# a16z/Lasso

Measured on AMD Instinct MI355X. Metric: prover lookups/sec for SparsePolynomialEvaluationProof, 2^24 AND lookups, higher is better.
Workload: dtype u256 (Montgomery Fr / ed25519 Fq integers)

## Files before the change

### lasso_amd/csrc/lasso_hip.hip

```cpp
#include <hip/hip_runtime.h>
#if defined(__SSE2__)
#include <emmintrin.h>
#endif
#include <mutex>
#include <string>
#include <unordered_map>
#include <vector>
#include <cstring>
#include <cstdio>
#include <cstdlib>
#include <ctime>
#include "../../include/lasso_hip.h"
#include "poly_kernels.cuh"
#include "msm_kernels.cuh"
#include "densify_kernels.cuh"

__global__ void __launch_bounds__(256) k_inner_lr(const fr_t* __restrict__ a, const fr_t* __restrict__ b, size_t half, fr_t* __restrict__ partials) {
  __shared__ RedScratch S;
  fr29 acc[3] = {fr29_zero(), fr29_zero(), fr29_zero()}; uint32_t cnt = 0;
  for (size_t i = blockIdx.x * (size_t)blockDim.x + threadIdx.x; i < half; i += (size_t)gridDim.x * blockDim.x) {
    acc[0] = fr29_weak(fr29_add(acc[0], fr29_mul(fr29_unpack_u(a[i]), fr29_unpack_s(b[half + i]))));
    acc[1] = fr29_weak(fr29_add(acc[1], fr29_mul(fr29_unpack_u(a[half + i]), fr29_unpack_s(b[i]))));
    if ((++cnt & 127u) == 0) { acc[0] = fr29_mul(acc[0], fr29_one_s()); acc[1] = fr29_mul(acc[1], fr29_one_s()); }
  }
  store_block_partials<3>(acc, 2, partials + 2 * (size_t)blockIdx.x, 0, S);
}

static_assert(sizeof(lasso_fr) == 32 && sizeof(fr_t) == 32, "Fr layout");
static_assert(sizeof(lasso_affine) == 64 && sizeof(lasso_point) == 128 && sizeof(ed_point) == 128 && sizeof(niels29) == (MSM_NIELS_ALIGN > 16 ? 128 : 112) && sizeof(pt29) == 144, "curve layouts");

struct EventPair { hipEvent_t a, b; int kid; double bytes, units, units2; bool large; bool counted; };
#define LASSO_PROF_COUNT_SLOTS 4096
struct lasso_ctx {
  int device = 0;
  hipStream_t stream = nullptr;
  std::string err;
  void* d_scratch = nullptr; size_t scratch_cap = 0;
  void* d_pip = nullptr; size_t pip_cap = 0;
  fr_t* d_small = nullptr;
  fr_t* h_small = nullptr;
  size_t small_cap = 0;
  uint32_t* h_flag = nullptr; uint32_t* d_flag = nullptr;
  uint32_t* h_tag = nullptr; uint32_t* d_tag = nullptr;
  bool tagged = true, pending_tagged = false;
  uint32_t pending_groups = 1, pending_K = 0;
  std::vector<lasso_fr> group_tmp;
  uint32_t* mail_h = nullptr; uint32_t* mail_d = nullptr;
  uint32_t seq = 0;
  uint64_t stat_waits = 0; double stat_wait_us = 0;
  fr_t* d_big = nullptr; fr_t* h_big = nullptr; size_t big_cap = 0;
  uint32_t* d_flags = nullptr;
  uint32_t* d_counters = nullptr;
  bool pending = false, defer_next = false; uint32_t pending_seq = 0; size_t pending_count = 0;
  bool ahead_active = false; uint32_t ahead_seq = 0; uint32_t* d_gmail = nullptr;
  bool tail_active = false; uint32_t tail_seq0 = 0, tail_turn = 0, tail_turns = 0; size_t tail_count = 0, tail_final = 0;
  bool tail_unstarted = false;
  uint32_t handover_next = 0;
  size_t ahead_count = 0; bool ahead_tagged = false; uint32_t ahead_groups = 1, ahead_K = 0; bool ahead_bullet = false;
  uint32_t* pmail_h = nullptr; uint32_t* pmail_d = nullptr; uint32_t* d_gpoint = nullptr;
  uint32_t gate_sent = 0;
  bool lay_active = false, lay_tail = false, lay_tagged = false, no_grow = false; uint32_t lay_seq = 0, lay_ell = 0, lay_groups = 1, lay_K = 0, lay_turns = 0; size_t lay_count = 0, lay_final = 0;
  uint32_t prof_mask = 0;
  std::vector<EventPair> events; size_t events_used = 0;
  uint64_t prof_launches[LASSO_K_COUNT] = {0}; double prof_ms[LASSO_K_COUNT] = {0}; double prof_bytes[LASSO_K_COUNT] = {0};
  uint64_t big_launches[LASSO_K_COUNT] = {0}; double big_ms[LASSO_K_COUNT] = {0}; double big_bytes[LASSO_K_COUNT] = {0};
  double prof_units[LASSO_K_COUNT] = {0}; double big_units[LASSO_K_COUNT] = {0};
  double prof_units2[LASSO_K_COUNT] = {0}; double big_units2[LASSO_K_COUNT] = {0};
  double prof_units3[LASSO_K_COUNT] = {0}; double big_units3[LASSO_K_COUNT] = {0};
  uint32_t* d_prof_counts = nullptr;
  void* rccl_comm = nullptr; int rccl_world = 0; int rccl_rank = -1;
  std::unordered_map<void*, size_t> mem_sizes; uint64_t mem_live = 0, mem_peak = 0; std::mutex mem_mu;
};
struct lasso_bases {
  size_t n = 0; niels29* d_table = nullptr;
  lasso_ctx* owner = nullptr;
  niels29* d_mult = nullptr;
  niels29* d_mult8 = nullptr;
  niels29* d_tab8[2] = {nullptr, nullptr};
  bool tab8_failed = false;
  std::mutex tab8_mu;
};

static thread_local std::string g_create_err;
static std::mutex g_ctx_mu; static std::vector<lasso_ctx*> g_ctx_live;
static lasso_ctx* live_or_null(lasso_ctx* c) { std::lock_guard<std::mutex> g(g_ctx_mu); for (lasso_ctx* x : g_ctx_live) if (x == c) return c; return nullptr; }

static int32_t fail(lasso_ctx* c, int32_t code, const std::string& msg) { if (c) c->err = msg; else g_create_err = msg; return code; }
#define HIPCHK(c, call) do { hipError_t e_ = (call); if (e_ != hipSuccess) return fail((c), e_ == hipErrorOutOfMemory ? LASSO_ERR_OOM : LASSO_ERR_HIP, std::string(#call) + ": " + hipGetErrorString(e_)); } while (0)
static inline bool bind_device(lasso_ctx* c) { if (!c) return true; int d = -1; if (hipGetDevice(&d) == hipSuccess && d == c->device) return true; return hipSetDevice(c->device) == hipSuccess; }
#define REQUIRE(c, cond) do { if (!bind_device(c)) return fail((c), LASSO_ERR_HIP, "hipSetDevice failed for the context's device"); \
                              if (!(cond)) return fail((c), LASSO_ERR_INVALID, std::string("invalid argument: ") + #cond); } while (0)

static hipError_t dmalloc(lasso_ctx* c, void** p, size_t bytes) {
  hipError_t e = hipMalloc(p, bytes);
  if (e == hipSuccess && c) { std::lock_guard<std::mutex> g(c->mem_mu); c->mem_sizes[*p] = bytes; c->mem_live += bytes; if (c->mem_live > c->mem_peak) c->mem_peak = c->mem_live; }
  return e;
}
static hipError_t dfree(lasso_ctx* c, void* p) {
  if (c && p) { std::lock_guard<std::mutex> g(c->mem_mu); auto it = c->mem_sizes.find(p); if (it != c->mem_sizes.end()) { c->mem_live -= it->second; c->mem_sizes.erase(it); } }
  return hipFree(p);
}

static int32_t ensure_scratch(lasso_ctx* c, size_t bytes) {
  if (bytes <= c->scratch_cap) return 0;
  if (c->no_grow) return LASSO_ERR_UNSUPPORTED;
  if (c->ahead_active || c->lay_active) return fail(c, LASSO_ERR_INVALID, "a launch is waiting on the device for its challenge: only lasso_result_wait and the post of that challenge are legal until then");
  if (c->d_scratch) { HIPCHK(c, hipStreamSynchronize(c->stream)); HIPCHK(c, dfree(c, c->d_scratch)); c->d_scratch = nullptr; c->scratch_cap = 0; }
  size_t cap = bytes < ((size_t)1 << 22) ? ((size_t)1 << 22) : bytes;
  HIPCHK(c, dmalloc(c, &c->d_scratch, cap)); c->scratch_cap = cap; return 0;
}
static int32_t ensure_pip(lasso_ctx* c, size_t bytes) {
  if (bytes <= c->pip_cap) return 0;
  if (c->no_grow || c->ahead_active || c->lay_active) return LASSO_ERR_UNSUPPORTED;
  if (c->d_pip) { HIPCHK(c, hipStreamSynchronize(c->stream)); HIPCHK(c, dfree(c, c->d_pip)); c->d_pip = nullptr; c->pip_cap = 0; }
  if (dmalloc(c, &c->d_pip, bytes) != hipSuccess) { (void)hipGetLastError(); c->d_pip = nullptr; return LASSO_ERR_UNSUPPORTED; }
  c->pip_cap = bytes; return 0;
}
static int32_t ensure_small(lasso_ctx* c, size_t count) {
  if (count <= c->small_cap) return 0;
  if (c->no_grow) return LASSO_ERR_UNSUPPORTED;
  if (c->ahead_active || c->lay_active) return fail(c, LASSO_ERR_INVALID, "a launch is waiting on the device for its challenge: only lasso_result_wait and the post of that challenge are legal until then");
  HIPCHK(c, hipStreamSynchronize(c->stream));
  if (c->h_small) (void)hipHostFree(c->h_small);
  c->h_small = nullptr; c->d_small = nullptr; c->small_cap = 0;
  size_t cap = count < 4096 ? 4096 : count;
  HIPCHK(c, hipHostMalloc((void**)&c->h_small, cap * sizeof(fr_t), hipHostMallocMapped | hipHostMallocCoherent));
  HIPCHK(c, hipHostGetDevicePointer((void**)&c->d_small, c->h_small, 0));
  if (c->h_tag) (void)hipHostFree(c->h_tag);
  c->h_tag = nullptr; c->d_tag = nullptr;
  HIPCHK(c, hipHostMalloc((void**)&c->h_tag, cap * 48, hipHostMallocMapped | hipHostMallocCoherent));
  memset(c->h_tag, 0, cap * 48);
  HIPCHK(c, hipHostGetDevicePointer((void**)&c->d_tag, c->h_tag, 0));
  c->small_cap = cap; return 0;
}
static int32_t ensure_big(lasso_ctx* c, size_t count) {
  if (count <= c->big_cap) return 0;
  if (c->no_grow) return LASSO_ERR_UNSUPPORTED;
  if (c->ahead_active || c->lay_active) return fail(c, LASSO_ERR_INVALID, "a launch is waiting on the device for its challenge: only lasso_result_wait and the post of that challenge are legal until then");
  HIPCHK(c, hipStreamSynchronize(c->stream));
  if (c->d_big) (void)dfree(c, c->d_big);
  if (c->h_big) (void)hipHostFree(c->h_big);
  c->d_big = nullptr; c->h_big = nullptr; c->big_cap = 0;
  size_t cap = count < 8192 ? 8192 : count;
  HIPCHK(c, dmalloc(c, (void**)&c->d_big, cap * sizeof(fr_t)));
// ... 224 lines not shown
  ncclResult_t r = a->AllGather(d_send, d_recv, bytes, ncclUint8, (ncclComm_t)c->rccl_comm, c->stream);
  if (r != ncclSuccess) return fail(c, LASSO_ERR_HIP, std::string("ncclAllGather: ") + a->GetErrorString(r));
  return 0;
}
int32_t lasso_points_reduce_compress(lasso_ctx* c, const void* d_parts, uint32_t groups, size_t rows, uint8_t* out32) {
  REQUIRE(c, d_parts && out32 && groups >= 1 && rows >= 1);
  int32_t rc = ensure_scratch(c, rows * 32 + 256); if (rc) return rc;
  {
    ProfScope ps(c, LASSO_K_MSM, (double)groups * rows * sizeof(pt29), (double)(groups - 1) * rows);
    hipLaunchKernelGGL(k_points_reduce_compress, dim3(grid_for(rows)), dim3(256), 0, c->stream, (const pt29*)d_parts, groups, rows, (uint32_t*)c->d_scratch);
  }
  HIPCHK(c, hipGetLastError());
  HIPCHK(c, hipMemcpyAsync(out32, c->d_scratch, rows * 32, hipMemcpyDeviceToHost, c->stream));
  HIPCHK(c, hipStreamSynchronize(c->stream));
  return 0;
}

static inline void mail_chunks(uint32_t* mail, uint32_t tag, const uint32_t w[8]) {
  const uint32_t chk = (w[0] ^ w[1] ^ w[2] ^ w[3] ^ w[4] ^ w[5] ^ w[6] ^ w[7]) + tag * 0x9E3779B9u;
#if defined(__SSE2__)
  _mm_store_si128((__m128i*)(mail + 0), _mm_set_epi32((int)w[2], (int)w[1], (int)w[0], (int)tag));
  _mm_store_si128((__m128i*)(mail + 4), _mm_set_epi32((int)w[5], (int)w[4], (int)w[3], (int)tag));
  _mm_store_si128((__m128i*)(mail + 8), _mm_set_epi32((int)chk, (int)w[7], (int)w[6], (int)tag));
#else
  const uint32_t m[12] = {tag, w[0], w[1], w[2], tag, w[3], w[4], w[5], tag, w[6], w[7], chk};
  for (int k : {1, 2, 3, 5, 6, 7, 9, 10, 11}) __atomic_store_n(mail + k, m[k], __ATOMIC_RELAXED);
  for (int k : {0, 4, 8}) __atomic_store_n(mail + k, m[k], __ATOMIC_RELEASE);
#endif
}
static inline void post_mail(lasso_ctx* c, uint32_t tag, const uint32_t w[8]) {
  mail_chunks(c->mail_h, tag, w);
#if defined(__SSE2__)
  _mm_sfence();
#else
  __atomic_thread_fence(__ATOMIC_SEQ_CST);
#endif
}
int32_t lasso_ctx_create(int32_t device, lasso_ctx** out) { return lasso_ctx_create_background(device, 0, out); }
int32_t lasso_ctx_device_uuid(lasso_ctx* c, uint8_t out[16]) {
  REQUIRE(c, c && out);
  hipUUID u; memset(&u, 0, sizeof(u));
  HIPCHK(c, hipDeviceGetUuid(&u, c->device));
  static_assert(sizeof(u.bytes) == 16, "hipUUID");
  memcpy(out, u.bytes, 16); return 0;
}
int32_t lasso_ctx_create_background(int32_t device, int32_t background, lasso_ctx** out) {
  if (!out) return fail(nullptr, LASSO_ERR_INVALID, "out is NULL");
  int n = 0;
  hipError_t e = hipGetDeviceCount(&n);
  if (e != hipSuccess || n == 0) return fail(nullptr, LASSO_ERR_HIP, std::string("no HIP device: ") + hipGetErrorString(e));
  if (device < 0 || device >= n) return fail(nullptr, LASSO_ERR_INVALID, "device index out of range");
  lasso_ctx* c = new lasso_ctx(); c->device = device;
  int prio_lo = 0, prio_hi = 0;
  if ((e = hipSetDevice(device)) == hipSuccess) (void)hipDeviceGetStreamPriorityRange(&prio_lo, &prio_hi);
  if (e != hipSuccess || (e = hipStreamCreateWithPriority(&c->stream, hipStreamNonBlocking, background ? prio_lo : prio_hi)) != hipSuccess) {
    std::string m = hipGetErrorString(e); delete c; return fail(nullptr, LASSO_ERR_HIP, m);
  }
  if (hipMalloc((void**)&c->d_flags, 64) != hipSuccess) { delete c; return fail(nullptr, LASSO_ERR_OOM, "flags alloc"); }
  if (hipMalloc((void**)&c->d_counters, (LASSO_MAX_PTRS + 40) * 4) != hipSuccess || hipMemset(c->d_counters, 0, (LASSO_MAX_PTRS + 40) * 4) != hipSuccess) { delete c; return fail(nullptr, LASSO_ERR_OOM, "counters alloc"); }
  if (hipHostMalloc((void**)&c->h_flag, 256, hipHostMallocMapped | hipHostMallocCoherent) != hipSuccess || hipHostGetDevicePointer((void**)&c->d_flag, c->h_flag, 0) != hipSuccess) { delete c; return fail(nullptr, LASSO_ERR_OOM, "mapped flag alloc"); }
  *c->h_flag = 0;
  { const char* v = getenv("LASSO_TAGGED_RESULTS"); c->tagged = !(v && v[0] == '0'); }
  { const char* v = getenv("LASSO_SEQ_START"); if (v) c->seq = (uint32_t)strtoul(v, nullptr, 0); }
  c->mail_h = c->h_flag + 32; c->mail_d = c->d_flag + 32;
  memset(c->h_flag, 0, 256);
  int32_t rc = ensure_small(c, (size_t)1 << 16); if (rc) { g_create_err = c->err; delete c; return rc; }
  rc = ensure_scratch(c, (size_t)1 << 22); if (rc) { g_create_err = c->err; delete c; return rc; }
  if (dmalloc(c, (void**)&c->d_gmail, 128) != hipSuccess || hipMemset(c->d_gmail, 0, 128) != hipSuccess) { g_create_err = "gmail alloc"; delete c; return LASSO_ERR_OOM; }
  if (hipHostMalloc((void**)&c->pmail_h, LASSO_PMAIL_BYTES, hipHostMallocMapped | hipHostMallocCoherent) != hipSuccess || hipHostGetDevicePointer((void**)&c->pmail_d, c->pmail_h, 0) != hipSuccess) { g_create_err = "point mailbox alloc"; delete c; return LASSO_ERR_OOM; }
  memset(c->pmail_h, 0, LASSO_PMAIL_BYTES);
  if (dmalloc(c, (void**)&c->d_gpoint, LASSO_GPOINT_BYTES) != hipSuccess || hipMemset(c->d_gpoint, 0, LASSO_GPOINT_BYTES) != hipSuccess) { g_create_err = "gpoint alloc"; delete c; return LASSO_ERR_OOM; }
  { std::lock_guard<std::mutex> g(g_ctx_mu); g_ctx_live.push_back(c); }
  *out = c; return 0;
}
int32_t lasso_abort(lasso_ctx* c) {
  REQUIRE(c, c);
  const uint32_t zero8[8] = {0, 0, 0, 0, 0, 0, 0, 0};
  if (c->lay_active && c->pmail_h) for (uint32_t j = 0; j < LASSO_POINT_MAX + 2; j++) mail_chunks(c->pmail_h + 12 * j, LASSO_MAIL_POISON, zero8);
  if (c->tail_active || c->ahead_active || c->lay_active) { mail_chunks(c->mail_h + 12, LASSO_MAIL_POISON, zero8); post_mail(c, LASSO_MAIL_POISON, zero8); }
  (void)hipStreamSynchronize(c->stream);
  (void)hipGetLastError();
  if (c->pmail_h) { memset(c->pmail_h, 0, LASSO_PMAIL_BYTES); c->gate_sent = 0; }
  mail_chunks(c->mail_h + 12, 0, zero8); post_mail(c, 0, zero8);
  c->lay_active = false; c->lay_tail = false; c->no_grow = false;
  c->ahead_active = false; c->ahead_bullet = false; c->tail_unstarted = false; c->handover_next = 0;
  c->tail_active = false; c->pending = false; c->defer_next = false; c->events_used = 0; c->pending_groups = 1; c->pending_K = 0;
  HIPCHK(c, hipMemsetAsync(c->d_counters, 0, (LASSO_MAX_PTRS + 40) * 4, c->stream));
  HIPCHK(c, hipStreamSynchronize(c->stream));
  return 0;
}
void lasso_ctx_destroy(lasso_ctx* c) {
  if (!c) return;
  { std::lock_guard<std::mutex> g(g_ctx_mu); for (size_t i = 0; i < g_ctx_live.size(); i++) if (g_ctx_live[i] == c) { g_ctx_live.erase(g_ctx_live.begin() + i); break; } }
  (void)hipSetDevice(c->device);
  if (c->tail_active || c->pending || c->ahead_active || c->lay_active) (void)lasso_abort(c);
  (void)hipStreamSynchronize(c->stream);
  rccl_release(c);
  for (auto& p : c->events) { (void)hipEventDestroy(p.a); (void)hipEventDestroy(p.b); }
  if (c->d_scratch) (void)hipFree(c->d_scratch);
  if (c->d_pip) (void)hipFree(c->d_pip);
  if (c->d_gmail) (void)hipFree(c->d_gmail);
  if (c->d_gpoint) (void)hipFree(c->d_gpoint);
  if (c->pmail_h) (void)hipHostFree(c->pmail_h);
  if (c->h_small) (void)hipHostFree(c->h_small);
  if (c->h_tag) (void)hipHostFree(c->h_tag);
  if (c->h_flag) (void)hipHostFree(c->h_flag);
  if (c->d_big) (void)hipFree(c->d_big);
  if (c->h_big) (void)hipHostFree(c->h_big);
  if (c->d_flags) (void)hipFree(c->d_flags);
  if (c->d_counters) (void)hipFree(c->d_counters);
  if (c->d_prof_counts) (void)hipFree(c->d_prof_counts);
  (void)hipStreamDestroy(c->stream);
  delete c;
}
const char* lasso_last_error(lasso_ctx* c) { return c ? c->err.c_str() : g_create_err.c_str(); }
void* lasso_stream(lasso_ctx* c) { return c ? (void*)c->stream : nullptr; }
int32_t lasso_alloc(lasso_ctx* c, size_t bytes, void** d_out) { REQUIRE(c, d_out); HIPCHK(c, dmalloc(c, d_out, bytes ? bytes : 1)); return 0; }
int32_t lasso_free(lasso_ctx* c, void* p) { if (!p) return 0; REQUIRE(c, c && !c->ahead_active && !c->lay_active); HIPCHK(c, hipStreamSynchronize(c->stream)); HIPCHK(c, dfree(c, p)); return 0; }
int32_t lasso_mem_stats(lasso_ctx* c, uint64_t* live_bytes, uint64_t* peak_bytes, int32_t reset_peak) {
  REQUIRE(c, c); std::lock_guard<std::mutex> g(c->mem_mu);
  if (live_bytes) *live_bytes = c->mem_live; if (peak_bytes) *peak_bytes = c->mem_peak; if (reset_peak) c->mem_peak = c->mem_live; return 0;
}
int32_t lasso_trim(lasso_ctx* c) {
  REQUIRE(c, c && !c->pending && !c->tail_active && !c->ahead_active && !c->lay_active);
  HIPCHK(c, hipStreamSynchronize(c->stream));
  if (c->d_pip) { HIPCHK(c, dfree(c, c->d_pip)); c->d_pip = nullptr; c->pip_cap = 0; }
  if (c->scratch_cap <= ((size_t)1 << 22)) return 0;
  HIPCHK(c, dfree(c, c->d_scratch)); c->d_scratch = nullptr; c->scratch_cap = 0;
  return ensure_scratch(c, (size_t)1 << 22);
}
int32_t lasso_upload(lasso_ctx* c, void* d, const void* s, size_t n) { REQUIRE(c, d && s && !c->ahead_active && !c->lay_active); HIPCHK(c, hipMemcpyAsync(d, s, n, hipMemcpyHostToDevice, c->stream)); HIPCHK(c, hipStreamSynchronize(c->stream)); return 0; }
int32_t lasso_download(lasso_ctx* c, void* d, const void* s, size_t n) { REQUIRE(c, d && s && !c->ahead_active && !c->lay_active); HIPCHK(c, hipMemcpyAsync(d, s, n, hipMemcpyDeviceToHost, c->stream)); HIPCHK(c, hipStreamSynchronize(c->stream)); return 0; }
int32_t lasso_copy(lasso_ctx* c, void* d, const void* s, size_t n) { REQUIRE(c, d && s); ProfScope ps(c, LASSO_K_MISC, 2.0 * n); HIPCHK(c, hipMemcpyAsync(d, s, n, hipMemcpyDeviceToDevice, c->stream)); return 0; }
int32_t lasso_zero(lasso_ctx* c, void* d, size_t n) { REQUIRE(c, d); HIPCHK(c, hipMemsetAsync(d, 0, n, c->stream)); return 0; }
int32_t lasso_sync(lasso_ctx* c) { REQUIRE(c, c && !c->ahead_active && !c->lay_active); HIPCHK(c, hipStreamSynchronize(c->stream)); return 0; }

int32_t lasso_prof_get_large(lasso_ctx* c, int32_t k, uint64_t* launches, double* ms, double* bytes) {
  REQUIRE(c, k >= 0 && k < LASSO_K_COUNT); prof_flush(c);
  if (launches) *launches = c->big_launches[k]; if (ms) *ms = c->big_ms[k]; if (bytes) *bytes = c->big_bytes[k]; return 0;
}
int32_t lasso_wait_stats(lasso_ctx* c, uint64_t* waits, double* wait_us, int32_t reset) { REQUIRE(c, waits && wait_us); *waits = c->stat_waits; *wait_us = c->stat_wait_us; if (reset) { c->stat_waits = 0; c->stat_wait_us = 0; } return 0; }
int32_t lasso_prof_enable(lasso_ctx* c, int32_t mask) { prof_flush(c); c->prof_mask = (uint32_t)mask; return 0; }
int32_t lasso_prof_reset(lasso_ctx* c) { prof_flush(c); for (int i = 0; i < LASSO_K_COUNT; i++) { c->prof_launches[i] = 0; c->prof_ms[i] = 0; c->prof_bytes[i] = 0; c->big_launches[i] = 0; c->big_ms[i] = 0; c->big_bytes[i] = 0; c->prof_units[i] = 0; c->big_units[i] = 0; c->prof_units2[i] = 0; c->big_units2[i] = 0; c->prof_units3[i] = 0; c->big_units3[i] = 0; } return 0; }
int32_t lasso_prof_get_units(lasso_ctx* c, int32_t k, int32_t large_only, double* units) {
  REQUIRE(c, k >= 0 && k < LASSO_K_COUNT && units); prof_flush(c);
  const bool large = large_only & 1, second = large_only & 2, third = large_only & 4;
  *units = third ? (large ? c->big_units3[k] : c->prof_units3[k]) : second ? (large ? c->big_units2[k] : c->prof_units2[k]) : (large ? c->big_units[k] : c->prof_units[k]); return 0;
}
int32_t lasso_prof_get(lasso_ctx* c, int32_t k, uint64_t* launches, double* ms, double* bytes) {
  REQUIRE(c, k >= 0 && k < LASSO_K_COUNT); prof_flush(c);
  if (launches) *launches = c->prof_launches[k]; if (ms) *ms = c->prof_ms[k]; if (bytes) *bytes = c->prof_bytes[k]; return 0;
}

int32_t lasso_fr_from_u32(lasso_ctx* c, const uint32_t* d_src, size_t n, lasso_fr* d_dst) {
  REQUIRE(c, d_src && d_dst); if (!n) return 0;
  ProfScope ps(c, LASSO_K_MISC, 36.0 * n);
  hipLaunchKernelGGL(k_from_u32, dim3(grid_for(n)), dim3(LASSO_BLOCK), 0, c->stream, d_src, n, (fr_t*)d_dst);
  HIPCHK(c, hipGetLastError()); return 0;
}
__global__ void __launch_bounds__(256) k_subtable_u32(int32_t kind, uint32_t sub, uint32_t log_m, uint32_t log_r, uint32_t* __restrict__ out) {
  const size_t m = (size_t)1 << log_m; const uint32_t bits = log_m / 2, mask = (1u << bits) - 1u;
  for (size_t i = blockIdx.x * (size_t)blockDim.x + threadIdx.x; i < m; i += (size_t)gridDim.x * blockDim.x) {
    const uint32_t r = (uint32_t)i & mask, l = (uint32_t)(i >> bits) & mask;
    uint32_t v;
    if (kind == LASSO_AND) v = l & r;
    else if (kind == LASSO_OR) v = l | r;
    else if (kind == LASSO_XOR) v = l ^ r;
// ... 215 lines not shown
static bool make_eq_inline(const lasso_fr* point, uint32_t ell, const lasso_fr* scale, EqInline& Q) {
  if (ell > 14 || (ell && !point)) return false;
  for (uint32_t j = 0; j < 14; j++) Q.r[j] = j < ell ? to_fr(point + j) : fr_zero();
  Q.scale = scale ? to_fr(scale) : fr_one(); Q.ell = ell; return true;
}
int32_t lasso_sumcheck_cubic_eqw2_begin_eq(lasso_ctx* c, lasso_fr* const* d_A, lasso_fr* const* d_B, uint32_t ncirc, lasso_fr* d_E_out, size_t n, const lasso_fr* point, uint32_t ell, const lasso_fr* scale) {
  REQUIRE(c, d_A && d_B && d_E_out && ncirc >= 1 && ncirc <= LASSO_MAX_PTRS && n >= 2 && (n & (n - 1)) == 0 && !c->pending && ((size_t)1 << ell) == n / 2);
  EqInline Q;
  if (n / 2 <= CUBIC_SMALL_Q || (ell && !point) || ell > 32) return fail(c, LASSO_ERR_UNSUPPORTED, "lasso_sumcheck_cubic_eqw2_begin_eq: tables of 2^7 .. 2^32 entries only");
  uint32_t seq, groups; int32_t rc;
  if (make_eq_inline(point, ell, scale, Q)) rc = cubic_eqw_launch(c, d_A, d_B, ncirc, d_E_out, n, nullptr, 2, &seq, &Q, &groups);
  else { EqPointArg G; G.point = point; G.ell = ell; G.scale = scale ? to_fr(scale) : fr_one(); rc = cubic_eqw_launch(c, d_A, d_B, ncirc, d_E_out, n, nullptr, 2, &seq, nullptr, &groups, false, &G); }
  if (rc) return rc;
  c->pending = true; c->pending_seq = seq; c->pending_count = (size_t)ncirc * 2; c->pending_tagged = c->tagged; c->pending_groups = groups; c->pending_K = 2;
  return 0;
}
int32_t lasso_sumcheck_cubic_tail_begin_eq(lasso_ctx* c, lasso_fr* const* d_A, lasso_fr* const* d_B, uint32_t ncirc, size_t n, const lasso_fr* point, uint32_t ell, const lasso_fr* scale) {
  const uint32_t ho = take_handover(c);
  REQUIRE(c, n >= 2 && ((size_t)1 << ell) == n / 2 && ell <= 9);
  EqInline Q; if (!make_eq_inline(point, ell, scale, Q)) return fail(c, LASSO_ERR_INVALID, "lasso_sumcheck_cubic_tail_begin_eq: bad point");
  return cubic_tail_begin_impl(c, ho, d_A, d_B, ncirc, nullptr, n, nullptr, &Q, false);
}
extern "C++" {
template <class TM>
static int32_t cubic_tail_begin_t(lasso_ctx* c, uint32_t m_stop_arg, lasso_fr* const* d_A, lasso_fr* const* d_B, uint32_t ncirc, const lasso_fr* d_E, size_t n, const lasso_fr* r, const EqInline* eqi, bool ahead, int gate_ell) {
  const uint32_t m_stop = m_stop_arg ? m_stop_arg : 1u;
  const bool gated = gate_ell >= 0;
  REQUIRE(c, d_A && d_B && (d_E || eqi || gated) && ncirc >= 1 && ncirc <= LASSO_MAX_PTRS && n >= ((r || ahead) ? 4u : 2u) && (n & (n - 1)) == 0 && (ahead || gated || !c->pending) && (gated || !c->tail_active) && !c->defer_next && !c->ahead_active && !c->lay_active);
  const size_t q = (r || ahead) ? n / 4 : n / 2;
  REQUIRE(c, q >= 1 && q <= CUBIC_TAIL_Q && (m_stop & (m_stop - 1)) == 0 && m_stop <= 128 && 2 * q > m_stop);
  TM A, B; for (uint32_t i = 0; i < ncirc; i++) { REQUIRE(c, d_A[i] && d_B[i]); A.p[i] = (fr_t*)d_A[i]; B.p[i] = (fr_t*)d_B[i]; }
  int32_t rc = ensure_small(c, (size_t)ncirc * 2 * (m_stop > 2 ? m_stop : 2)); if (rc) return rc;
  uint32_t turns = 0; while (((size_t)m_stop << turns) < 2 * q) turns++;
  const uint32_t seq0 = next_seq(c, turns + 1);
#define LAUNCH_CTAIL(B_, Q_, I_, TE_, R_, EQ_) hipLaunchKernelGGL((k_cubic_tail<B_, Q_, I_, TM, TE_>), dim3(ncirc), dim3(Q_), 0, c->stream, A, B, (const fr_t*)d_E, (uint32_t)q, R_, (const uint32_t*)c->mail_d, c->d_counters, RES(c), seq0, EQ_, m_stop, ahead ? 1u : 0u)
  if (gated) {
    hipLaunchKernelGGL(k_gate_point, dim3(1), dim3(64), 0, c->stream, (const uint32_t*)c->pmail_d, c->d_gpoint, seq0, (uint32_t)gate_ell + 2u, c->pmail_d + LASSO_PMAIL_ACK_WORD); c->gate_sent = seq0;
    EqInlineMem M; M.gp = c->d_gpoint; M.seq = seq0; M.ell = (uint32_t)gate_ell;
    if (q <= 256) LAUNCH_CTAIL(false, 256, true, EqInlineMem, fr_zero(), M); else LAUNCH_CTAIL(false, 512, true, EqInlineMem, fr_zero(), M);
    HIPCHK(c, hipGetLastError());
    c->lay_active = true; c->lay_tail = true; c->lay_seq = seq0; c->lay_ell = (uint32_t)gate_ell; c->lay_turns = turns; c->lay_count = (size_t)ncirc * 2; c->lay_final = (size_t)ncirc * 2 * m_stop; c->lay_tagged = c->tagged;
    return 0;
  }
  if (eqi) { if (q <= 256) LAUNCH_CTAIL(false, 256, true, EqInline, fr_zero(), *eqi); else LAUNCH_CTAIL(false, 512, true, EqInline, fr_zero(), *eqi); }
  else if (q <= 256) { if (r || ahead) LAUNCH_CTAIL(true, 256, false, EqNone, r ? to_fr(r) : fr_zero(), EqNone()); else LAUNCH_CTAIL(false, 256, false, EqNone, fr_zero(), EqNone()); }
  else { if (r || ahead) LAUNCH_CTAIL(true, 512, false, EqNone, r ? to_fr(r) : fr_zero(), EqNone()); else LAUNCH_CTAIL(false, 512, false, EqNone, fr_zero(), EqNone()); }
  HIPCHK(c, hipGetLastError());
  c->tail_active = true; c->tail_seq0 = seq0; c->tail_turn = 0; c->tail_turns = turns; c->tail_count = (size_t)ncirc * 2; c->tail_final = (size_t)ncirc * 2 * m_stop;
  if (ahead) { c->tail_unstarted = true; return 0; }
  c->pending = true; c->pending_seq = seq0; c->pending_count = c->tail_count; c->pending_tagged = c->tagged;
  return 0;
}
}
static int32_t cubic_tail_begin_impl(lasso_ctx* c, uint32_t m_stop, lasso_fr* const* d_A, lasso_fr* const* d_B, uint32_t ncirc, const lasso_fr* d_E, size_t n, const lasso_fr* r, const EqInline* eqi, bool ahead, int gate_ell) {
  return ncirc <= 8 ? cubic_tail_begin_t<MutPtrTable8>(c, m_stop, d_A, d_B, ncirc, d_E, n, r, eqi, ahead, gate_ell) : cubic_tail_begin_t<MutPtrTable>(c, m_stop, d_A, d_B, ncirc, d_E, n, r, eqi, ahead, gate_ell);
}
static bool gate_free(lasso_ctx* c) { return !c->gate_sent || __atomic_load_n(c->pmail_h + LASSO_PMAIL_ACK_WORD, __ATOMIC_ACQUIRE) == c->gate_sent; }
int32_t lasso_layer_ahead_ok(lasso_ctx* c) { static const bool off = [] { const char* v = getenv("LASSO_LAYER_AHEAD"); return v && v[0] == '0'; }(); return c && !off && c->pmail_d && c->d_gpoint ? 1 : 0; }
int32_t lasso_sumcheck_cubic_eqw2_begin_eq_ahead(lasso_ctx* c, lasso_fr* const* d_A, lasso_fr* const* d_B, uint32_t ncirc, lasso_fr* d_E_out, size_t n, uint32_t ell) {
  REQUIRE(c, d_A && d_B && d_E_out && ncirc >= 1 && ncirc <= LASSO_MAX_PTRS && n >= 2 && (n & (n - 1)) == 0 && ell < 48 && ((size_t)1 << ell) == n / 2 && !c->lay_active && !c->ahead_active && !c->defer_next);
  if (!lasso_layer_ahead_ok(c) || n / 2 <= CUBIC_SMALL_Q || ell > 32 || ell > LASSO_POINT_MAX) return fail(c, LASSO_ERR_UNSUPPORTED, "lasso_sumcheck_cubic_eqw2_begin_eq_ahead: tables of 2^7 .. 2^32 entries only");
  if (!gate_free(c)) return fail(c, LASSO_ERR_UNSUPPORTED, "lasso_sumcheck_cubic_eqw2_begin_eq_ahead: the previous point gate has not consumed its message yet");
  uint32_t seq, groups;
  c->no_grow = true;
  const int32_t rc = cubic_eqw_launch(c, d_A, d_B, ncirc, d_E_out, n, nullptr, 2, &seq, nullptr, &groups, false, nullptr, (int)ell);
  c->no_grow = false;
  if (rc == LASSO_ERR_UNSUPPORTED) return fail(c, rc, "lasso_sumcheck_cubic_eqw2_begin_eq_ahead: a buffer would have to grow while kernels are in flight");
  if (rc) return rc;
  HIPCHK(c, hipGetLastError());
  c->lay_active = true; c->lay_tail = false; c->lay_seq = seq; c->lay_ell = ell; c->lay_count = (size_t)ncirc * 2; c->lay_tagged = c->tagged; c->lay_groups = groups; c->lay_K = 2;
  return 0;
}
int32_t lasso_sumcheck_cubic_tail_begin_eq_ahead(lasso_ctx* c, lasso_fr* const* d_A, lasso_fr* const* d_B, uint32_t ncirc, size_t n, uint32_t ell) {
  const uint32_t ho = take_handover(c);
  REQUIRE(c, n >= 2 && ell <= 9 && ((size_t)1 << ell) == n / 2);
  if (!lasso_layer_ahead_ok(c)) return fail(c, LASSO_ERR_UNSUPPORTED, "lasso_sumcheck_cubic_tail_begin_eq_ahead: switched off");
  if (!gate_free(c)) return fail(c, LASSO_ERR_UNSUPPORTED, "lasso_sumcheck_cubic_tail_begin_eq_ahead: the previous point gate has not consumed its message yet");
  c->no_grow = true;
  const int32_t rc = cubic_tail_begin_impl(c, ho, d_A, d_B, ncirc, nullptr, n, nullptr, nullptr, false, (int)ell);
  c->no_grow = false;
  if (rc == LASSO_ERR_UNSUPPORTED) return fail(c, rc, "lasso_sumcheck_cubic_tail_begin_eq_ahead: a buffer would have to grow while kernels are in flight");
  return rc;
}
static void point_mail(lasso_ctx* c, uint32_t ell, const lasso_fr* point, const lasso_fr* scale, uint32_t ctrl) {
  const uint32_t zero8[8] = {0, 0, 0, 0, 0, 0, 0, 0}; const fr_t one = fr_one();
  for (uint32_t j = 0; j < ell; j++) mail_chunks(c->pmail_h + 12 * j, c->lay_seq, point ? (const uint32_t*)(point + j) : zero8);
  mail_chunks(c->pmail_h + 12 * ell, c->lay_seq, scale ? (const uint32_t*)scale : one.v);
  const uint32_t ctl[8] = {ctrl, 0, 0, 0, 0, 0, 0, 0};
  mail_chunks(c->pmail_h + 12 * (ell + 1), c->lay_seq, ctl);
#if defined(__SSE2__)
  _mm_sfence();
#else
  __atomic_thread_fence(__ATOMIC_SEQ_CST);
#endif
}
int32_t lasso_point_post(lasso_ctx* c, const lasso_fr* point, uint32_t ell, const lasso_fr* scale) {
  REQUIRE(c, c && c->lay_active && ell == c->lay_ell && (point || !ell) && !c->pending && !c->tail_active && !c->ahead_active);
  point_mail(c, ell, point, scale, 0u);
  c->lay_active = false;
  if (c->lay_tail) {
    c->tail_active = true; c->tail_seq0 = c->lay_seq; c->tail_turn = 0; c->tail_turns = c->lay_turns; c->tail_count = c->lay_count; c->tail_final = c->lay_final; c->tail_unstarted = false;
    c->pending = true; c->pending_seq = c->lay_seq; c->pending_count = c->lay_count; c->pending_tagged = c->lay_tagged; c->pending_groups = 1; c->pending_K = 0;
  } else {
    c->pending = true; c->pending_seq = c->lay_seq; c->pending_count = c->lay_count; c->pending_tagged = c->lay_tagged; c->pending_groups = c->lay_groups; c->pending_K = c->lay_K;
  }
  c->lay_tail = false;
  return 0;
}
int32_t lasso_point_cancel(lasso_ctx* c) {
  REQUIRE(c, c && c->lay_active);
  point_mail(c, c->lay_ell, nullptr, nullptr, 1u);
  c->lay_active = false; c->lay_tail = false;
  return 0;
}
int32_t lasso_sumcheck_cubic_tail_begin_ahead(lasso_ctx* c, lasso_fr* const* d_A, lasso_fr* const* d_B, uint32_t ncirc, const lasso_fr* d_E, size_t n) {
  const uint32_t ho = take_handover(c);
  REQUIRE(c, d_E);
  return cubic_tail_begin_impl(c, ho, d_A, d_B, ncirc, d_E, n, nullptr, nullptr, true);
}
int32_t lasso_tail_handover_next(lasso_ctx* c, uint32_t m_stop) {
  REQUIRE(c, c && (m_stop & (m_stop - 1)) == 0 && m_stop <= 128);
  c->handover_next = m_stop <= 1 ? 0 : m_stop; return 0;
}
int32_t lasso_sumcheck_linear_tail_begin(lasso_ctx* c, const lasso_fr* const* d_src, uint32_t alpha, const lasso_fr* d_E, size_t n, const lasso_fr* r) {
  const uint32_t ho = take_handover(c);
  REQUIRE(c, d_src && d_E && alpha >= 1 && alpha <= LASSO_MAX_PTRS && n >= (r ? 4u : 2u) && (n & (n - 1)) == 0 && !c->pending && !c->tail_active && !c->defer_next && !ho && !c->ahead_active);
  const size_t q = r ? n / 4 : n / 2;
  REQUIRE(c, q >= 1 && q <= CUBIC_TAIL_Q);
  PtrTable Src; for (uint32_t i = 0; i < alpha; i++) { REQUIRE(c, d_src[i]); Src.p[i] = (const fr_t*)d_src[i]; }
  int32_t rc = ensure_small(c, (size_t)alpha * 3); if (rc) return rc;
  uint32_t turns = 0; while (((size_t)1 << turns) < 2 * q) turns++;
  const uint32_t seq0 = next_seq(c, turns + 1);
#define LAUNCH_LTAIL(B_, Q_, R_) hipLaunchKernelGGL((k_linear_tail<B_, Q_>), dim3(alpha), dim3(Q_), 0, c->stream, Src, (const fr_t*)d_E, (uint32_t)q, R_, (const uint32_t*)c->mail_d, c->d_counters, RES(c), seq0)
  if (q <= 256) { if (r) LAUNCH_LTAIL(true, 256, to_fr(r)); else LAUNCH_LTAIL(false, 256, fr_zero()); }
  else { if (r) LAUNCH_LTAIL(true, 512, to_fr(r)); else LAUNCH_LTAIL(false, 512, fr_zero()); }
  HIPCHK(c, hipGetLastError());
  c->tail_active = true; c->tail_seq0 = seq0; c->tail_turn = 0; c->tail_turns = turns; c->tail_count = (size_t)alpha * 2; c->tail_final = alpha;
  c->pending = true; c->pending_seq = seq0; c->pending_count = c->tail_count; c->pending_tagged = c->tagged;
  return 0;
}
int32_t lasso_sumcheck_cubic_tail_next(lasso_ctx* c, const lasso_fr* r) {
  REQUIRE(c, r && c->tail_active && !c->pending);
  const fr_t rr = to_fr(r);
  if (c->tail_unstarted) {
    c->tail_unstarted = false;
    post_mail(c, c->tail_seq0, rr.v);
    c->pending = true; c->pending_seq = c->tail_seq0; c->pending_count = c->tail_count; c->pending_tagged = c->tagged;
    return 0;
  }
  c->tail_turn++;
  const uint32_t tn = c->tail_seq0 + c->tail_turn;
  post_mail(c, tn, rr.v);
  const size_t cnt = c->tail_turn == c->tail_turns ? c->tail_final : c->tail_count;
  if (cnt) { c->pending = true; c->pending_seq = c->tail_seq0 + c->tail_turn; c->pending_count = cnt; c->pending_tagged = c->tagged; }
  if (c->tail_turn == c->tail_turns) c->tail_active = false;
  return 0;
}
uint32_t lasso_sumcheck_tail_capacity(void) { static const uint32_t q = [] { const char* v = getenv("LASSO_TAIL_Q"); const long x = v ? atol(v) : 0; return (uint32_t)(x == 256 ? 256 : CUBIC_TAIL_Q); }(); return q; }
int32_t lasso_defer_next(lasso_ctx* c) { REQUIRE(c, !c->pending && !c->defer_next); c->defer_next = true; return 0; }
int32_t lasso_result_wait(lasso_ctx* c, lasso_fr* out, size_t count) {
  REQUIRE(c, out && c->pending && count == c->pending_count);
  c->pending = false;
  { const uint32_t g = c->pending_groups, K = c->pending_K; c->pending_groups = 1; c->pending_K = 0; return wait_flag(c, c->pending_seq, count, out, c->pending_tagged, g, K); }
}
int32_t lasso_sumcheck_linear_eqw_round(lasso_ctx* c, const lasso_fr* const* d_polys, uint32_t alpha, const lasso_fr* d_E, size_t n, lasso_fr* out) {
  REQUIRE(c, d_polys && d_E && out && alpha >= 1 && alpha <= LASSO_MAX_PTRS && n >= 2 && (n & (n - 1)) == 0);
  PtrTable P; for (uint32_t i = 0; i < alpha; i++) { REQUIRE(c, d_polys[i]); P.p[i] = (const fr_t*)d_polys[i]; }
  const size_t half = n / 2; const unsigned ny = alpha, nx = grid_for(half, cubic_nx_cap(ny));
  int32_t rc = ensure_small(c, (size_t)alpha * 3); if (rc) return rc;
  rc = ensure_scratch(c, (size_t)nx * ny * 3 * sizeof(fr_t)); if (rc) return rc;
  const uint32_t seq = next_seq(c);
  {
    ProfScope ps(c, LASSO_K_COMBINE, 32.0 * n * (alpha + 1.0));
    hipLaunchKernelGGL(k_dot_eqw_lb, dim3(nx * ny), dim3(LASSO_BLOCK), 0, c->stream, P, nx, ny, (const fr_t*)d_E, half, (fr_t*)c->d_scratch, c->d_counters, RES(c), seq);
  }
  HIPCHK(c, hipGetLastError());
  return wait_flag(c, seq, (size_t)alpha * 3, out, c->tagged);
}
int32_t lasso_sumcheck_linear_eqw_round_fused(lasso_ctx* c, lasso_fr* const* d_polys, uint32_t alpha, const lasso_fr* d_E, size_t n, const lasso_fr* r, lasso_fr* out) {
  return lasso_sumcheck_linear_eqw_round_fused_from(c, (const lasso_fr* const*)d_polys, d_polys, alpha, d_E, n, r, out);
}
int32_t lasso_sumcheck_linear_eqw_round_fused_from(lasso_ctx* c, const lasso_fr* const* d_src, lasso_fr* const* d_polys, uint32_t alpha, const lasso_fr* d_E, size_t n, const lasso_fr* r, lasso_fr* out) {
  REQUIRE(c, d_src && d_polys && d_E && r && out && alpha >= 1 && alpha <= LASSO_MAX_PTRS && n >= 4 && (n & (n - 1)) == 0);
  MutPtrTable P; PtrTable Src; for (uint32_t i = 0; i < alpha; i++) { REQUIRE(c, d_polys[i] && d_src[i]); P.p[i] = (fr_t*)d_polys[i]; Src.p[i] = (const fr_t*)d_src[i]; }
  const size_t q = n / 4; const unsigned ny = alpha, nx = grid_for(q, cubic_nx_cap(ny));
  int32_t rc = ensure_small(c, (size_t)alpha * 3); if (rc) return rc;
  rc = ensure_scratch(c, (size_t)nx * ny * 3 * sizeof(fr_t)); if (rc) return rc;
  const uint32_t seq = next_seq(c);
  {
    ProfScope ps(c, LASSO_K_BIND, 48.0 * n * (alpha + 1.0));
    hipLaunchKernelGGL(k_dot_eqw_fused<false>, dim3(nx * ny), dim3(LASSO_BLOCK), 0, c->stream, Src, P, nx, ny, (const fr_t*)d_E, q, to_fr(r), (fr_t*)c->d_scratch, c->d_counters, RES(c), seq);
  }
  HIPCHK(c, hipGetLastError());
  return wait_flag(c, seq, (size_t)alpha * 3, out, c->tagged);
}
// ... 787 lines not shown
```

### lasso_amd/csrc/poly_kernels.cuh

```cuda
#pragma once
#define LASSO_MAIL_POISON 0xFFFFFFFFu
#include <hip/hip_runtime.h>
#include "fr.cuh"
#include "fr29.cuh"

#ifndef LASSO_MAX_PTRS
#define LASSO_MAX_PTRS 136
#endif
#define LASSO_BLOCK 256
#define LASSO_MAX_ALPHA 32

struct PtrTable { const fr_t* p[LASSO_MAX_PTRS]; };
struct MutPtrTable { fr_t* p[LASSO_MAX_PTRS]; };
struct PtrTable8 { const fr_t* p[8]; };
struct MutPtrTable8 { fr_t* p[8]; };
struct StrategyDev { int kind; uint32_t c, log_m, log_r, alpha; };
struct WeightTable { fr_t w[LASSO_MAX_ALPHA]; };

struct RedScratch { int32_t rows[LASSO_BLOCK * 27]; int64_t strips[8 * 27]; int64_t cols[27]; };
template <int NV>
__device__ __forceinline__ void block_columns(const fr29* vals, RedScratch& S) {
  const uint32_t t = threadIdx.x;
  __syncthreads();
#pragma unroll
// ... 45 lines not shown
#pragma unroll
      for (int k = 0; k < 4; k++) __hip_atomic_store(o + k, (uint64_t)v.v[2 * k] | ((uint64_t)v.v[2 * k + 1] << 32), __ATOMIC_RELAXED, __HIP_MEMORY_SCOPE_AGENT);
      return;
    }
#endif
    out[slot] = v;
  }
}
__device__ __forceinline__ bool mail_valid(const lasso_u32x4& c0, const lasso_u32x4& c1, const lasso_u32x4& c2, uint32_t tag) {
  return c0.x == tag && c1.x == tag && c2.x == tag && c2.w == (c0.y ^ c0.z ^ c0.w ^ c1.y ^ c1.z ^ c1.w ^ c2.y ^ c2.z) + tag * 0x9E3779B9u;
}
__device__ __forceinline__ bool mail_wait(const uint32_t* mailbox, uint32_t tag, uint64_t t_end, fr_t& chal) {
  const lasso_u32x4* m4 = reinterpret_cast<const lasso_u32x4*>(mailbox);
  lasso_u32x4 c0, c1, c2; uint32_t spins = 0;
  for (;;) {
#ifndef LASSO_NO_POLL_FENCE
    __builtin_amdgcn_fence(__ATOMIC_ACQUIRE, "");
#else
    asm volatile("" ::: "memory");
#endif
    c0 = __builtin_nontemporal_load(m4); c1 = __builtin_nontemporal_load(m4 + 1); c2 = __builtin_nontemporal_load(m4 + 2);
    if (mail_valid(c0, c1, c2, tag)) break;
    if (c0.x == LASSO_MAIL_POISON || ((++spins & 63u) == 0 && wall_clock64() > t_end)) return false;
  }
  chal.v[0] = c0.y; chal.v[1] = c0.z; chal.v[2] = c0.w; chal.v[3] = c1.y; chal.v[4] = c1.z; chal.v[5] = c1.w; chal.v[6] = c2.y; chal.v[7] = c2.z;
  return true;
}
__global__ void __launch_bounds__(64) k_gate(const uint32_t* mail, uint32_t* gmail, uint32_t seq, uint32_t pair) {
  if (threadIdx.x != 0) return;
  const uint64_t t_end = wall_clock64() + 500000000ull;
  fr_t c0, c1;
  bool ok = mail_wait(mail, seq, t_end, c0);
  if (ok && pair) ok = mail_wait(mail + 12, seq, t_end, c1);
  if (ok) {
#pragma unroll
    for (int k = 0; k < 8; k++) { gmail[k] = c0.v[k]; if (pair) gmail[8 + k] = c1.v[k]; }
    gmail[16] = seq;
  } else gmail[17] = seq;
}
__device__ __forceinline__ bool ahead_challenge(const uint32_t* mail, uint32_t* gmail, uint32_t seq, fr_t& r, uint32_t* s_mail) {
  if (threadIdx.x == 0) {
    const uint64_t t_end = wall_clock64() + 500000000ull;
    uint32_t ok = 1, spins = 0;
    if (blockIdx.x == 0) {
      fr_t c;
      if (mail_wait(mail, seq, t_end, c)) {
#pragma unroll
        for (int k = 0; k < 8; k++) gmail[k] = c.v[k];
        __builtin_amdgcn_fence(__ATOMIC_RELEASE, "agent");
        __hip_atomic_store(gmail + 16, seq, __ATOMIC_RELEASE, __HIP_MEMORY_SCOPE_AGENT);
      } else __hip_atomic_store(gmail + 17, seq, __ATOMIC_RELEASE, __HIP_MEMORY_SCOPE_AGENT);
    }
    for (;;) {
      if (__hip_atomic_load(gmail + 16, __ATOMIC_ACQUIRE, __HIP_MEMORY_SCOPE_AGENT) == seq) break;
      if (__hip_atomic_load(gmail + 17, __ATOMIC_ACQUIRE, __HIP_MEMORY_SCOPE_AGENT) == seq || ((++spins & 63u) == 0 && wall_clock64() > t_end + 100000000ull)) { ok = 0; break; }
      __builtin_amdgcn_s_sleep(8);
    }
    if (ok) {
#pragma unroll
      for (int k = 0; k < 8; k++) s_mail[k] = __hip_atomic_load(gmail + k, __ATOMIC_RELAXED, __HIP_MEMORY_SCOPE_AGENT);
    }
    s_mail[8] = ok;
  }
  __syncthreads();
  if (!s_mail[8]) return false;
#pragma unroll
  for (int k = 0; k < 8; k++) r.v[k] = s_mail[k];
  return true;
}
__device__ __forceinline__ bool gated_challenge(const uint32_t* gmail, uint32_t seq, uint32_t words, uint32_t* s_mail) {
  if (threadIdx.x < 17) {
    const uint32_t t = threadIdx.x;
    if (t < words) s_mail[t] = gmail[t];
    if (t == 16) s_mail[16] = (gmail[16] == seq && gmail[17] != seq) ? 1u : 0u;
  }
  __syncthreads();
  return s_mail[16] != 0;
}
#define LASSO_POINT_MAX 40
#define LASSO_GP_TAG (8 * (LASSO_POINT_MAX + 2))
#define LASSO_PMAIL_BYTES 2048
#define LASSO_GPOINT_BYTES 2048
#define LASSO_PMAIL_ACK_WORD 504
__global__ void __launch_bounds__(64) k_gate_point(const uint32_t* pmail, uint32_t* gpoint, uint32_t seq, uint32_t nfr, uint32_t* ack) {
  const uint32_t t = threadIdx.x;
  const uint64_t t_end = wall_clock64() + 500000000ull;
  bool ok = true; fr_t v = fr_zero();
  if (t < nfr) {
    ok = mail_wait(pmail + 12 * t, seq, t_end, v);
    if (ok) {
#pragma unroll
      for (int k = 0; k < 8; k++) gpoint[8 * t + k] = v.v[k];
      if (t == nfr - 1 && v.v[0] != 0) ok = false;
    }
  }
  const bool all_ok = __ballot(!ok) == 0;
  __builtin_amdgcn_fence(__ATOMIC_RELEASE, "agent");
  if (t == 0) { gpoint[LASSO_GP_TAG + (all_ok ? 0 : 1)] = seq; if (ack) __hip_atomic_store(ack, seq, __ATOMIC_RELEASE, __HIP_MEMORY_SCOPE_SYSTEM); }
}
__device__ __forceinline__ bool gate_point_ok(const uint32_t* __restrict__ gp, uint32_t seq) { return gp[LASSO_GP_TAG] == seq && gp[LASSO_GP_TAG + 1] != seq; }
__device__ __forceinline__ fr_t gate_point_fr(const uint32_t* __restrict__ gp, uint32_t j) {
  fr_t r;
#pragma unroll
  for (int k = 0; k < 8; k++) r.v[k] = gp[8 * j + k];
  return r;
}
template <int KMAX>
__device__ __forceinline__ void store_block_partials(const fr29* acc, uint32_t K, fr_t* __restrict__ dst, int shift, RedScratch& S, uint32_t* flag = nullptr, uint32_t seq = 0, size_t slot0 = 0) {
#pragma unroll
  for (int k0 = 0; k0 < KMAX; k0 += 3) if ((uint32_t)k0 < K) {
    fr29 grp[3];
#pragma unroll
    for (int v = 0; v < 3; v++) grp[v] = (k0 + v < KMAX) ? acc[(k0 + v < KMAX) ? k0 + v : 0] : fr29_zero();
    block_columns<3>(grp, S);
    if (threadIdx.x < 3 && k0 + threadIdx.x < K) result_store(dst, slot0 + k0 + threadIdx.x, columns_to_fr(S, threadIdx.x, shift), flag, seq);
  }
}

__device__ __forceinline__ void reduce_partials_row(const fr_t* __restrict__ partials, uint32_t nx, uint32_t K, uint32_t y, fr_t* __restrict__ out, RedScratch& S, uint32_t Kv = 0xffffffffu,
                                                    uint32_t* flag = nullptr, uint32_t seq = 0) {
  if (Kv > K) Kv = K;
  for (uint32_t k0 = 0; k0 < Kv; k0 += 3) {
    fr29 acc[3];
#pragma unroll
    for (int v = 0; v < 3; v++) {
      acc[v] = fr29_zero();
      if (k0 + v < Kv) for (uint32_t x = threadIdx.x; x < nx; x += blockDim.x) acc[v] = fr29_weak(fr29_add(acc[v], fr29_unpack_u(partials[((size_t)y * nx + x) * K + k0 + v])));
    }
    block_columns<3>(acc, S);
    if (threadIdx.x < 3 && k0 + threadIdx.x < Kv) result_store(out, (size_t)y * K + k0 + threadIdx.x, columns_to_fr(S, threadIdx.x, 0), flag, seq);
  }
}
__global__ void __launch_bounds__(LASSO_BLOCK) k_reduce_partials(const fr_t* __restrict__ partials, uint32_t nx, uint32_t K, fr_t* __restrict__ out) {
  __shared__ RedScratch S;
  reduce_partials_row(partials, nx, K, blockIdx.x, out, S);
}

__device__ __forceinline__ void row_done(uint32_t nrows, uint32_t* counters, uint32_t* flag, uint32_t seq);
__device__ __forceinline__ void last_block_reduce(const fr_t* partials, uint32_t nx, uint32_t K, uint32_t y, uint32_t nrows, uint32_t* counters, fr_t* __restrict__ out, RedScratch& S,
                                                  uint32_t* flag, uint32_t seq, uint32_t Kv = 0xffffffffu) {
  __shared__ uint32_t is_last;
  if (threadIdx.x == 0) {
#ifdef LASSO_PLAIN_PARTIALS
    __builtin_amdgcn_fence(__ATOMIC_RELEASE, "agent");
#endif
    asm volatile("s_waitcnt vmcnt(0)" ::: "memory");
    uint32_t ticket = __hip_atomic_fetch_add(&counters[y], 1u, __ATOMIC_RELAXED, __HIP_MEMORY_SCOPE_AGENT);
    uint32_t last = (ticket == nx - 1) ? 1u : 0u;
    if (last) { __builtin_amdgcn_fence(__ATOMIC_ACQUIRE, "agent"); counters[y] = 0; }
    is_last = last;
  }
  __syncthreads();
  if (!is_last) return;
  reduce_partials_row(partials, nx, K, y, out, S, Kv, flag, seq);
  row_done(nrows, counters, flag, seq);
}

__global__ void __launch_bounds__(LASSO_BLOCK) k_bind_top(MutPtrTable polys, size_t half, fr_t r) {
  fr_t* __restrict__ z = polys.p[blockIdx.y];
  const fr29 rs = fr29_unpack_s(r);
  for (size_t i = blockIdx.x * (size_t)blockDim.x + threadIdx.x; i < half; i += (size_t)gridDim.x * blockDim.x) {
    const fr29 lo = fr29_unpack_u(z[i]), hi = fr29_unpack_u(z[i + half]);
    z[i] = fr29_store(fr29_add(lo, fr29_mul(fr29_sub(hi, lo), rs)));
  }
}

__device__ __forceinline__ void cubic_terms(const fr29& a0, const fr29& a1, const fr29& b0, const fr29& b1, const fr29& c0, const fr29& c1, fr29& t0, fr29& t2, fr29& t3) {
  t0 = fr29_mul(c0, fr29_mul(a0, b0));
  const fr29 da = fr29_sub(a1, a0), db = fr29_sub(b1, b0), dc = fr29_sub(c1, c0);
  const fr29 a2 = fr29_weak(fr29_add(a1, da)), b2 = fr29_weak(fr29_add(b1, db)), c2 = fr29_weak(fr29_add(c1, dc));
  t2 = fr29_mul(c2, fr29_mul(a2, b2));
  const fr29 a3 = fr29_add(a2, da), b3 = fr29_weak(fr29_add(b2, db)), c3 = fr29_add(c2, dc);
  t3 = fr29_mul(c3, fr29_mul(a3, b3));
}
struct CubicGrid { uint32_t bx, by, nx, ny; };
__device__ __forceinline__ CubicGrid cubic_grid(uint32_t nx, uint32_t ny) {
  CubicGrid g; g.nx = nx; g.ny = ny;
  const uint32_t b = blockIdx.x;
  if ((nx & 7u) == 0) { const uint32_t grp = b / (8 * ny), r = b - grp * 8 * ny; g.by = r >> 3; g.bx = grp * 8 + (r & 7u); }
  else { g.bx = b % nx; g.by = b / nx; }
  return g;
// ... 96 lines not shown
    fr29 p = one_s;
    for (uint32_t j = 0; j < lb; j++) { const bool bit = (x >> (lb - 1 - j)) & 1u; const fr29 rs = fr29_unpack_s(eq_point_r(Q, hb + j)); p = fr29_mul(bit ? rs : fr29_sub(one_s, rs), p); }
    T.lo_s[x] = p;
    T.lo_u[x] = fr29_mul(p, fr29_unpack_u(fr_one()));
  }
  __syncthreads();
  return true;
}
__device__ __forceinline__ bool eq_inline_build(const EqInline& Q, EqInlineTables& T) { return eq_inline_build_t(Q, T); }
__device__ __forceinline__ bool eq_inline_build(const EqInlineMem& Q, EqInlineTables& T) { return eq_inline_build_t(Q, T); }
__device__ __forceinline__ fr29 eq_inline_s(const EqInlineTables& T, uint32_t lb, size_t x) { return fr29_mul(T.hi_s[x >> lb], T.lo_s[x & ((1u << lb) - 1u)]); }
struct EqGlobal { const fr_t* hi; const fr_t* lo; uint32_t lo_bits; uint32_t ell; const uint32_t* gp; uint32_t seq; };
__device__ __forceinline__ bool eq_inline_build(const EqGlobal& Q, EqInlineTables&) { return Q.gp == nullptr || gate_point_ok(Q.gp, Q.seq); }
__device__ __forceinline__ bool eq_inline_build(const EqNone&, EqInlineTables&) { return true; }
template <class TE> __device__ __forceinline__ bool eq_gate_ok(const TE&) { return true; }
template <> __device__ __forceinline__ bool eq_gate_ok<EqNone>(const EqNone& Q) { return Q.gp == nullptr || gate_point_ok(Q.gp, Q.seq); }
__device__ __forceinline__ fr29 eq_inline_value(const EqInline&, const EqInlineTables& T, uint32_t lb, size_t i, bool write, fr_t* __restrict__ E_out) {
  if (write) E_out[i] = fr29_store(fr29_mul(T.hi_s[i >> lb], T.lo_u[i & ((1u << lb) - 1u)]));
  return eq_inline_s(T, lb, i);
}
__device__ __forceinline__ fr29 eq_inline_value(const EqInlineMem&, const EqInlineTables& T, uint32_t lb, size_t i, bool write, fr_t* __restrict__ E_out) {
  if (write) E_out[i] = fr29_store(fr29_mul(T.hi_s[i >> lb], T.lo_u[i & ((1u << lb) - 1u)]));
  return eq_inline_s(T, lb, i);
}
__device__ __forceinline__ fr29 eq_inline_value(const EqGlobal& Q, const EqInlineTables&, uint32_t, size_t i, bool write, fr_t* __restrict__ E_out) {
  const fr_t mem = fr29_store(fr29_mul(fr29_unpack_u(Q.hi[i >> Q.lo_bits]), fr29_unpack_s(Q.lo[i & (((size_t)1 << Q.lo_bits) - 1)])));
  if (write) E_out[i] = mem;
  return fr29_unpack_s(mem);
}
__device__ __forceinline__ fr29 eq_inline_value(const EqNone&, const EqInlineTables&, uint32_t, size_t, bool, fr_t* __restrict__) { return fr29_zero(); }
__device__ __forceinline__ fr_t fr_load_nt(const fr_t* p) {
  const lasso_u32x4* q = reinterpret_cast<const lasso_u32x4*>(p);
  const lasso_u32x4 x = __builtin_nontemporal_load(q), y = __builtin_nontemporal_load(q + 1);
  fr_t r; r.v[0] = x.x; r.v[1] = x.y; r.v[2] = x.z; r.v[3] = x.w; r.v[4] = y.x; r.v[5] = y.y; r.v[6] = y.z; r.v[7] = y.w; return r;
}
template <int NT, bool EQI = false, class TP = PtrTable, class TE = EqInline, bool NTL = false>
__global__ void __launch_bounds__(LASSO_BLOCK) k_cubic_eqw_lb(TP A, TP B, uint32_t nx, uint32_t ny, const fr_t* __restrict__ E, size_t half, fr_t* __restrict__ partials, uint32_t* counters,
                                                               fr_t* __restrict__ out, uint32_t* flag, uint32_t seq, uint32_t pipeline, TE EQ = TE(), fr_t* __restrict__ E_out = nullptr) {
  __shared__ RedScratch S;
  __shared__ EqInlineTables ET;
  const CubicGrid g = cubic_grid(nx, ny);
  const uint32_t elb = EQ.ell / 2;
  if constexpr (EQI) { if (!eq_inline_build(EQ, ET)) return; } else { if (!eq_gate_ok(EQ)) return; }
  const fr_t* __restrict__ a = A.p[g.by];
  const fr_t* __restrict__ b = B.p[g.by];
  fr29 e[3] = {fr29_zero(), fr29_zero(), fr29_zero()}; uint32_t cnt = 0;
  fr29_acc w0 = fr29_acc_zero(), w1 = fr29_acc_zero();
  const size_t stride = (size_t)nx * blockDim.x;
  size_t i = g.bx * (size_t)blockDim.x + threadIdx.x;
  if (NT == 3) {
    for (; i < half; i += stride) {
      fr29 t0, t2, t3;
      cubic_eqw_terms(fr29_unpack_u(a[i]), fr29_unpack_u(a[i + half]), fr29_unpack_u(b[i]), fr29_unpack_u(b[i + half]), fr29_unpack_s(E[i]), t0, t2, t3); CUBIC_ACCUMULATE(e, t0, t2, t3, cnt);
    }
  } else if (!pipeline) {
    for (; i < half; i += stride) {
      const fr29 es = fr29_unpack_s(E[i]), b0 = fr29_unpack_u(b[i]), b1 = fr29_unpack_u(b[i + half]);
      const fr29 g0 = fr29_mul(fr29_unpack_u(a[i]), es), g1 = fr29_mul(fr29_unpack_u(a[i + half]), es);
      fr29_mul_acc(w0, b0, g0); fr29_mul_acc(w1, fr29_sub(g1, g0), fr29_sub(b1, b0));
      if (++cnt == 3) { fr29_acc_carry(w0); fr29_acc_carry(w1); cnt = 0; }
    }
  } else if (i < half) {
#define LB_LD(ptr) (NTL ? fr_load_nt(ptr) : *(ptr))
    fr_t a0 = LB_LD(a + i), a1 = LB_LD(a + i + half), b0m = LB_LD(b + i), b1m = LB_LD(b + i + half), em = EQI ? fr_zero() : E[i];
    for (;;) {
      const size_t in = i + stride; const bool more = in < half;
      const size_t ip = more ? in : i;
      const fr_t na0 = LB_LD(a + ip), na1 = LB_LD(a + ip + half), nb0 = LB_LD(b + ip), nb1 = LB_LD(b + ip + half), ne = EQI ? fr_zero() : E[ip];
#undef LB_LD
      fr29 es;
      if (EQI) es = eq_inline_value(EQ, ET, elb, i, g.by == 0, E_out);
      else es = fr29_unpack_s(em);
      const fr29 b0 = fr29_unpack_u(b0m), b1 = fr29_unpack_u(b1m);
      const fr29 g0 = fr29_mul(fr29_unpack_u(a0), es), g1 = fr29_mul(fr29_unpack_u(a1), es);
      fr29_mul_acc(w0, b0, g0); fr29_mul_acc(w1, fr29_sub(g1, g0), fr29_sub(b1, b0));
      if (++cnt == 3) { fr29_acc_carry(w0); fr29_acc_carry(w1); cnt = 0; }
      if (!more) break;
      a0 = na0; a1 = na1; b0m = nb0; b1m = nb1; em = ne; i = in;
    }
  }
  if (NT == 2) { fr29_acc_carry(w0); fr29_acc_carry(w1); e[0] = fr29_acc_reduce(w0); e[1] = fr29_acc_reduce(w1); }
  cubic_epilogue(e, g, partials, counters, out, flag, seq, S, 5, NT);
}
template <int NT, bool WIDE = false, class TM = MutPtrTable, bool AHEAD = false>
#ifdef LASSO_FUSED_WAVES
__attribute__((amdgpu_waves_per_eu(LASSO_FUSED_WAVES, LASSO_FUSED_WAVES)))
#endif
__global__ void __launch_bounds__(LASSO_BLOCK) k_cubic_eqw_fused(TM A, TM B, uint32_t nx, uint32_t ny, const fr_t* __restrict__ E, size_t q, fr_t r,
                                                                  fr_t* __restrict__ partials, uint32_t* counters, fr_t* __restrict__ out, uint32_t* flag, uint32_t seq,
                                                                  const uint32_t* gmail = nullptr, const uint32_t* mail = nullptr) {
  __shared__ RedScratch S;
  const CubicGrid g = cubic_grid(nx, ny);
  fr_t* __restrict__ a = A.p[g.by];
  fr_t* __restrict__ b = B.p[g.by];
  if constexpr (AHEAD) {
    __shared__ uint32_t s_mail[17];
    if (mail) {
      if (!ahead_challenge(mail, const_cast<uint32_t*>(gmail), seq, r, s_mail)) return;
    } else {
      if (!gated_challenge(gmail, seq, 8, s_mail)) return;
#pragma unroll
      for (int k = 0; k < 8; k++) r.v[k] = s_mail[k];
    }
  }
  const fr29 rs = fr29_unpack_s(r);
  fr29 e[3] = {fr29_zero(), fr29_zero(), fr29_zero()}; uint32_t cnt = 0;
  fr29_acc w0 = fr29_acc_zero(), w1 = fr29_acc_zero();
  for (size_t i = g.bx * (size_t)blockDim.x + threadIdx.x; i < q; i += (size_t)nx * blockDim.x) {
    const fr29 a0 = NT == 2 ? bind29_semi(a[i], a[i + 2 * q], rs) : bind29(a[i], a[i + 2 * q], rs), a1 = NT == 2 ? bind29_semi(a[i + q], a[i + 3 * q], rs) : bind29(a[i + q], a[i + 3 * q], rs);
    a[i] = fr29_pack(a0); a[i + q] = fr29_pack(a1);
    const fr29 b0 = NT == 2 ? bind29_semi(b[i], b[i + 2 * q], rs) : bind29(b[i], b[i + 2 * q], rs), b1 = NT == 2 ? bind29_semi(b[i + q], b[i + 3 * q], rs) : bind29(b[i + q], b[i + 3 * q], rs);
    b[i] = fr29_pack(b0); b[i + q] = fr29_pack(b1);
    fr29 t0, t2, t3;
    if (NT == 3) { cubic_eqw_terms(a0, a1, b0, b1, fr29_unpack_s(E[i]), t0, t2, t3); CUBIC_ACCUMULATE(e, t0, t2, t3, cnt); }
    else if (!WIDE) { cubic_eqw_terms2(a0, a1, b0, b1, fr29_unpack_s(E[i]), t0, t2); CUBIC_ACCUMULATE2(e, t0, t2, cnt); }
    else {
      const fr29 es = fr29_unpack_s(E[i]);
      const fr29 g0 = fr29_mul(a0, es), g1 = fr29_mul(a1, es);
      fr29_mul_acc(w0, b0, g0); fr29_mul_acc(w1, fr29_sub(g1, g0), fr29_sub(b1, b0));
      if (++cnt == 3) { fr29_acc_carry(w0); fr29_acc_carry(w1); cnt = 0; }
    }
  }
  if (WIDE && NT == 2) { fr29_acc_carry(w0); fr29_acc_carry(w1); e[0] = fr29_acc_reduce(w0); e[1] = fr29_acc_reduce(w1); }
  cubic_epilogue(e, g, partials, counters, out, flag, seq, S, 5, NT);
}
template <bool BIND, int NT, class TM = MutPtrTable>
__global__ void __launch_bounds__(LASSO_BLOCK) k_cubic_eqw_small(TM A, TM B, const fr_t* __restrict__ E, uint32_t q, fr_t r, uint32_t* counters, fr_t* __restrict__ out,
                                                                  uint32_t* flag, uint32_t seq) {
  __shared__ fr29 bound[2][128];
  __shared__ fr29 ge[128];
  __shared__ int32_t rows[192 * 9];
  __shared__ int64_t cols[27];
  const uint32_t t = threadIdx.x, y = blockIdx.x, m = 2 * q;
  const fr29 rs = fr29_unpack_s(r);
  for (uint32_t item = t; item < 2 * m; item += LASSO_BLOCK) {
    const uint32_t p = item / m, i = item - p * m;
    fr_t* dst = p == 0 ? A.p[y] : B.p[y];
    fr29 v;
    if (BIND) { v = bind29(dst[i], dst[i + m], rs); dst[i] = fr29_pack(v); } else v = fr29_unpack_u(dst[i]);
    bound[p][i] = v;
  }
  __syncthreads();
  if (t < m) ge[t] = fr29_mul(bound[0][t], fr29_unpack_s(E[t < q ? t : t - q]));
  __syncthreads();
  const uint32_t x = t >> 6, i = t & 63;
  if (x < NT) {
    fr29 term = fr29_zero();
    if (i < q) {
      const fr29 g0 = ge[i], g1 = ge[i + q], b0 = bound[1][i], b1 = bound[1][i + q];
      if (x == 0) term = fr29_mul(b0, g0);
      else if (NT == 2) term = fr29_mul(fr29_sub(g1, g0), fr29_sub(b1, b0));
      else {
        const fr29 dg = fr29_sub(g1, g0), db = fr29_sub(b1, b0);
        const fr29 g2 = fr29_weak(fr29_add(g1, dg)), b2 = fr29_weak(fr29_add(b1, db));
        term = x == 1 ? fr29_mul(b2, g2) : fr29_mul(fr29_add(b2, db), fr29_weak(fr29_add(g2, dg)));
      }
    }
#pragma unroll
    for (int k = 0; k < 9; k++) rows[t * 9 + k] = term.v[k];
  }
  __syncthreads();
  if (t < 9 * NT) {
    const uint32_t v = t / 9, k = t - v * 9;
    int64_t sum = 0;
    for (uint32_t j = 0; j < 64; j++) sum += rows[(v * 64 + j) * 9 + k];
    cols[t] = sum;
// ... 729 lines not shown
```

### lasso_amd/host/prover.hpp

```cpp
#pragma once
#include <array>
#include <functional>
#include <map>
#include <memory>
#include <string>
#include <vector>
#include "field_host.hpp"
#include "field52.hpp"
#include "hashes.hpp"
#include "../../include/lasso_prover.h"

#include <chrono>
#include <cstdio>
#include <cstdlib>

namespace lasso {

struct Trace {
  static bool on() { static const bool v = [] { const char* e = getenv("LASSO_TRACE"); return e && e[0] == '1'; }(); return v; }
  static bool mem() { static const bool v = [] { const char* e = getenv("LASSO_TRACE"); return e && e[0] == '3'; }(); return v; }
  const char* name; lasso_ctx* ctx; std::chrono::steady_clock::time_point t0; static int& depth() { static thread_local int d = 0; return d; }
  uint64_t w0 = 0; double wus0 = 0; uint64_t live0 = 0;
  Trace(const char* n, lasso_ctx* c) : name(n), ctx(c) {
    if (on()) { t0 = std::chrono::steady_clock::now(); depth()++; if (ctx) lasso_wait_stats(ctx, &w0, &wus0, 0); }
    if (mem() && ctx) { uint64_t pk = 0; lasso_mem_stats(ctx, &live0, &pk, 1); depth()++; }
  }
  ~Trace() {
    if (mem() && ctx) {
      uint64_t live = 0, pk = 0; lasso_mem_stats(ctx, &live, &pk, 1); depth()--;
      fprintf(stderr, "[mem] %*s%s: live at entry %.2f GB, peak inside %.2f GB, live at exit %.2f GB\n", 2 * depth(), "", name, live0 / 1e9, pk / 1e9, live / 1e9);
    }
    if (!on()) return;
    if (ctx) lasso_sync(ctx);
    depth()--;
    double ms = std::chrono::duration<double, std::milli>(std::chrono::steady_clock::now() - t0).count();
    uint64_t w1 = 0; double wus1 = 0; if (ctx) lasso_wait_stats(ctx, &w1, &wus1, 0);
    fprintf(stderr, "[trace] %*s%s: time.busy=%.3fms (device hand-offs %llu, host spinning %.3fms)\n", 2 * depth(), "", name, ms, (unsigned long long)(w1 - w0), (wus1 - wus0) * 1e-3);
  }
};

struct HostClock {
  static bool on() { static const bool v = [] { const char* e = getenv("LASSO_TRACE"); return e && e[0] == '2'; }(); return v; }
  static std::map<std::string, double>& buckets() { static thread_local std::map<std::string, double> b; return b; }
  const char* name; std::chrono::steady_clock::time_point t0;
  explicit HostClock(const char* n) : name(n) { if (on()) t0 = std::chrono::steady_clock::now(); }
  ~HostClock() { if (on()) buckets()[name] += std::chrono::duration<double, std::milli>(std::chrono::steady_clock::now() - t0).count(); }
  static void dump() { if (!on()) return; for (auto& kv : buckets()) fprintf(stderr, "[host] %-28s %.3f ms\n", kv.first.c_str(), kv.second); buckets().clear(); }
};
struct Error : std::runtime_error { using std::runtime_error::runtime_error; };
#define LASSO_REQUIRE(c) do { if (!(c)) throw Error(std::string("lasso prover: requirement failed: ") + #c); } while (0)

#define LASSO_HOST_TOPS_MAX_PTRS 128
inline size_t next_pow2(size_t n) { size_t p = 1; while (p < n) p <<= 1; return p; }
inline bool is_pow2(size_t n) { return n && !(n & (n - 1)); }
inline size_t ceil_log2(size_t n) { size_t k = 0; while (((size_t)1 << k) < n) k++; return k; }

typedef int32_t (*lasso_allgather_fn)(void* user, const void* send, void* recv, size_t bytes);
struct Comm {
  size_t rank = 0, world = 1; lasso_allgather_fn fn = nullptr; void* user = nullptr;
  bool shared_device = false;
  bool sharded() const { return world > 1; }
  size_t log_world() const { size_t k = 0; while (((size_t)1 << k) < world) k++; return k; }
  void allgather(const void* send, void* recv, size_t bytes) const {
    if (world == 1) { memcpy(recv, send, bytes); return; }
    if (!fn || fn(user, send, recv, bytes) != 0) throw std::runtime_error("lasso prover: all-gather failed");
  }
  void sum(std::vector<lasso_fr>& v) const {
    if (world == 1 || v.empty()) return;
    std::vector<lasso_fr> all(v.size() * world);
    allgather(v.data(), all.data(), v.size() * sizeof(lasso_fr));
    for (size_t i = 0; i < v.size(); i++) { Sc acc = Sc::zero(); for (size_t g = 0; g < world; g++) acc += Sc::from_abi(all[g * v.size() + i]); v[i] = acc.abi(); }
  }
  Sc eq_low(const ScVec& point) const {
    const size_t p = log_world(); Sc f = Sc::one();
    for (size_t b = 0; b < p; b++) { const Sc& rv = point[point.size() - 1 - b]; f *= ((rank >> b) & 1) ? rv : (Sc::one() - rv); }
    return f;
  }
};

class Dev {
  mutable std::multimap<size_t, void*> pool_;
  mutable std::map<void*, size_t> live_;
  mutable size_t in_use_ = 0, in_use_peak_ = 0;
  int device_ = 0;
  mutable lasso_ctx* side_ = nullptr;

 public:
  lasso_ctx* ctx = nullptr;
  Comm comm;
  bool capacity = [] { const char* e = getenv("LASSO_CAPACITY"); return e && e[0] == '1'; }();
  bool throughput = false;
  bool no_ahead() const { static const bool keep = [] { const char* e = getenv("LASSO_THROUGHPUT_AHEAD"); return e && e[0] == '1'; }(); return throughput && !keep; }
// ... 453 lines not shown
  size_t s_loc, m_loc;
  std::vector<DBufU32> dim_u32;
  DBuf combined_l_variate_polys, combined_log_m_variate_polys;
  size_t nv_l, nv_m;
  bool compact = false;
  std::vector<DBufU32> read_u32; std::vector<uint32_t> read_max;
  const lasso_fr* dim(size_t i) const { LASSO_REQUIRE(!compact); return combined_l_variate_polys.p + i * s_loc; }
  const lasso_fr* read(size_t i) const { LASSO_REQUIRE(!compact); return combined_l_variate_polys.p + (C + i) * s_loc; }
  const uint32_t* block_u32(size_t b) const { return b < C ? dim_u32[b].p : read_u32[b - C].p; }
  uint32_t block_max(size_t b) const { return b < C ? (uint32_t)(m - 1) : read_max[b - C]; }
  void lift_block(size_t b, lasso_fr* d_tmp) const { dev->chk(lasso_fr_from_u32(dev->ctx, block_u32(b), s_loc, d_tmp), "lasso_fr_from_u32"); }
  const lasso_fr* final_(size_t i) const { return combined_log_m_variate_polys.p + i * m_loc; }

  static std::unique_ptr<DensifiedRepresentation> from_lookup_indices(const Dev& d, const uint64_t* indices, size_t n_lookups, size_t C, size_t log_m) {
    Trace tr_all("DensifiedRepresentation.from_lookup_indices", d.ctx);
    auto D = std::make_unique<DensifiedRepresentation>();
    D->dev = &d; D->C = C; D->s = next_pow2(n_lookups); D->log_m = log_m; D->m = (size_t)1 << log_m;
    const size_t s = D->s, m = D->m, P = d.comm.world;
    if (d.comm.sharded() && (s < 2 * P || m < 2 * P)) throw Error("slab sharding needs at least 2 lookups and 2 table entries per rank");
    D->s_loc = s / P; D->m_loc = m / P;
    size_t n_l = next_pow2(2 * C * s), n_m = next_pow2(C) * m;
    D->nv_l = ceil_log2(n_l); D->nv_m = ceil_log2(n_m);
    if (d.comm.sharded() && (((size_t)1 << (D->nv_m - D->nv_m / 2)) < P || ((size_t)1 << (D->nv_l - D->nv_l / 2)) < P)) throw Error("slab sharding needs every Hyrax matrix to have at least one column per rank");
    D->compact = d.capacity && !capacity_compact_off() && D->s_loc >= capacity_leafless_min() && s >= ((size_t)1 << (D->nv_l - D->nv_l / 2));
    D->combined_log_m_variate_polys = DBuf(d, n_m / P);
    if (!D->compact) D->combined_l_variate_polys = DBuf(d, n_l / P);
    if (!D->compact && n_l > 2 * C * s) d.chk(lasso_zero(d.ctx, D->combined_l_variate_polys.p + 2 * C * D->s_loc, (n_l - 2 * C * s) / P * sizeof(lasso_fr)), "lasso_zero");
    if (n_m > C * m) d.chk(lasso_zero(d.ctx, D->combined_log_m_variate_polys.p + C * D->m_loc, (n_m - C * m) / P * sizeof(lasso_fr)), "lasso_zero");
    DBufU64 d_idx(d, indices, n_lookups * C);
    DBuf tmp_dim, tmp_read; if (D->compact) { tmp_dim = DBuf(d, D->s_loc); tmp_read = DBuf(d, D->s_loc); }
    for (size_t i = 0; i < C; i++) {
      DBufU32 d_access(d, D->s_loc);
      lasso_fr* dim_out = D->compact ? tmp_dim.p : D->combined_l_variate_polys.p + i * D->s_loc;
      lasso_fr* read_out = D->compact ? tmp_read.p : D->combined_l_variate_polys.p + (C + i) * D->s_loc;
      d.chk(lasso_densify_dim_slab(d.ctx, d_idx.p, n_lookups, C, i, s, (uint32_t)log_m, (uint32_t)P, (uint32_t)d.comm.rank, d_access.p, dim_out, read_out, D->combined_log_m_variate_polys.p + i * D->m_loc), "lasso_densify_dim");
      D->dim_u32.push_back(std::move(d_access));
      if (D->compact) {
        DBufU32 r32(d, D->s_loc); uint32_t mx = 0;
        d.chk(lasso_fr_to_u32(d.ctx, tmp_read.p, D->s_loc, r32.p, &mx), "lasso_fr_to_u32");
        D->read_u32.push_back(std::move(r32)); D->read_max.push_back(mx);
      }
    }
    if (D->compact) { tmp_dim.release(); tmp_read.release(); }
    if (d.capacity) (void)lasso_trim(d.ctx);
    return D;
  }
  SparsePolynomialCommitment commit(const SparsePolyCommitmentGens& gens) const {
    Trace tr_all("DensifiedRepresentation.commit", dev->ctx);
    SparsePolynomialCommitment c;
    if (!compact) c.l_variate_polys_commitment = hyrax_commit(*dev, combined_l_variate_polys.p, nv_l, gens.gens_combined_l_variate);
    else {
      const size_t L = (size_t)1 << (nv_l / 2), R = (size_t)1 << (nv_l - nv_l / 2), rows_per = s / R;
      PolyCommitment& pc = c.l_variate_polys_commitment; pc.rows = L; pc.compressed.reserve(32 * L);
      DBuf tmp(*dev, s_loc);
      for (size_t b = 0; b < 2 * C; b++) {
        PolyCommitment part;
        if (!dev->comm.sharded()) part = hyrax_commit_rows(*dev, nullptr, rows_per, R, gens.gens_combined_l_variate, block_u32(b), block_max(b));
        else { lift_block(b, tmp.p); part = hyrax_commit_rows(*dev, tmp.p, rows_per, R, gens.gens_combined_l_variate); }
        pc.compressed.insert(pc.compressed.end(), part.compressed.begin(), part.compressed.end());
      }
      if (2 * C * rows_per < L) {
        dev->chk(lasso_zero(dev->ctx, tmp.p, (R / dev->comm.world) * sizeof(lasso_fr)), "lasso_zero");
        PolyCommitment zero_row = hyrax_commit_rows(*dev, tmp.p, 1, R, gens.gens_combined_l_variate);
        for (size_t r = 2 * C * rows_per; r < L; r++) pc.compressed.insert(pc.compressed.end(), zero_row.compressed.begin(), zero_row.compressed.end());
      }
      tmp.release();
    }
    c.log_m_variate_polys_commitment = hyrax_commit(*dev, combined_log_m_variate_polys.p, nv_m, gens.gens_combined_log_m_variate);
    c.s = s; c.log_m = log_m; c.m = m; return c;
  }
};

class Prover {
  const Dev& d; const Strategy S; DensifiedRepresentation& dense; const SparsePolyCommitmentGens& gens; ProofTranscript& t; RandomTape& tape;
  size_t alpha, s, m, nv_derefs;
  size_t P, lgP, s_loc, m_loc;
  std::vector<DBuf> tables;
  DBuf combined_E;
  const lasso_fr* E(size_t i) const { return combined_E.p + i * s_loc; }
  std::vector<DBuf> tail_bufs;
  std::vector<DBuf> side_keep;
  static size_t tail_q() { static const size_t q = lasso_sumcheck_tail_capacity(); return q; }
  struct LazyEq { bool on = false; std::vector<lasso_fr> rr; lasso_fr scale; lasso_fr* d_table = nullptr; } lazy_eq;
  struct LayerAhead { bool on = false, tail = false; std::vector<lasso_fr*> A, B; lasso_fr* d_table = nullptr; size_t len = 0, m_stop = 1; uint32_t ell = 0; } layer_ahead;
  std::function<void()> next_layer_hook;
  static bool tail_switched_off() { static const bool off = [] { const char* v = getenv("LASSO_CUBIC_TAIL"); return v && v[0] == '0'; }(); return off; }
  bool layer_ahead_ok() { return P == 1 && !d.no_ahead() && !eq_inline_off() && !tail_switched_off() && lasso_layer_ahead_ok(d.ctx) == 1; }
  void enqueue_layer_ahead(const std::vector<lasso_fr*>& A, const std::vector<lasso_fr*>& B, size_t len, lasso_fr* d_table) {
    layer_ahead.on = false;
    if (!layer_ahead_ok() || len < 4) return;
    const size_t k = A.size(); const uint32_t ell = (uint32_t)ceil_log2(len / 2);
    LayerAhead la; la.A = A; la.B = B; la.d_table = d_table; la.len = len; la.ell = ell;
    int32_t rc;
    if (len / 2 <= tail_q()) {
      if (ell > 9) return;
      const size_t m0 = host_m_stop(k); la.m_stop = (m0 >= 2 && m0 < len) ? m0 : 1; la.tail = true;
      if (la.m_stop > 1) d.chk(lasso_tail_handover_next(d.ctx, (uint32_t)la.m_stop), "lasso_tail_handover_next");
      rc = lasso_sumcheck_cubic_tail_begin_eq_ahead(d.ctx, la.A.data(), la.B.data(), (uint32_t)k, len, ell);
    } else {
      if (ell > 32 || len / 2 <= 64) return;
      rc = lasso_sumcheck_cubic_eqw2_begin_eq_ahead(d.ctx, la.A.data(), la.B.data(), (uint32_t)k, d_table, len, ell);
    }
    if (rc == LASSO_ERR_UNSUPPORTED) return;
    d.chk(rc, "lasso_sumcheck_cubic_*_begin_eq_ahead");
    la.on = true; layer_ahead = std::move(la);
  }
  static bool eq_inline_off() { static const bool v = [] { const char* e = getenv("LASSO_EQ_INLINE"); return e && e[0] == '0'; }(); return v; }
  static bool side_off() { static const bool v = [] { const char* e = getenv("LASSO_SIDE_STREAM"); return e && e[0] == '0'; }(); return v; }

 public:
  std::vector<uint8_t> proof_bytes;
  Prover(const Dev& d_, const Strategy& S_, DensifiedRepresentation& dense_, const SparsePolyCommitmentGens& gens_, ProofTranscript& t_, RandomTape& tape_)
      : d(d_), S(S_), dense(dense_), gens(gens_), t(t_), tape(tape_) {
    alpha = S.num_memories(); s = dense.s; m = dense.m; LASSO_REQUIRE(S.C() == dense.C && S.M() == dense.m);
    P = d.comm.world; lgP = d.comm.log_world(); s_loc = dense.s_loc; m_loc = dense.m_loc;
  }

  void eq_evals_local(const ScVec& point, lasso_fr* d_out) {
    LASSO_REQUIRE(point.size() >= lgP);
    std::vector<lasso_fr> rr; for (size_t i = 0; i + lgP < point.size(); i++) rr.push_back(point[i].abi());
    if (P == 1) { d.chk(lasso_eq_evals(d.ctx, rr.data(), (uint32_t)rr.size(), d_out), "lasso_eq_evals"); return; }
    lasso_fr sc = d.comm.eq_low(point).abi();
    d.chk(lasso_eq_evals_scaled(d.ctx, rr.data(), (uint32_t)rr.size(), &sc, d_out), "lasso_eq_evals_scaled");
  }
  void eq_half_local(const ScVec& point, lasso_fr* d_out) {
    LASSO_REQUIRE(point.size() >= lgP);
    if (point.size() == lgP) return;
    std::vector<lasso_fr> rr; for (size_t i = 1; i + lgP < point.size(); i++) rr.push_back(point[i].abi());
    Sc scale = Sc::one() - point[0]; if (P > 1) scale *= d.comm.eq_low(point);
    lasso_fr sc = scale.abi();
    d.chk(lasso_eq_evals_scaled(d.ctx, rr.data(), (uint32_t)rr.size(), &sc, d_out), "lasso_eq_evals_scaled");
  }
  void eq_half_lazy(const ScVec& point, lasso_fr* d_out) {
    LASSO_REQUIRE(point.size() >= lgP);
    lazy_eq.on = false;
    if (point.size() == lgP) return;
    lazy_eq.rr.clear(); for (size_t i = 1; i + lgP < point.size(); i++) lazy_eq.rr.push_back(point[i].abi());
    Sc scale = Sc::one() - point[0]; if (P > 1) scale *= d.comm.eq_low(point);
    lazy_eq.scale = scale.abi(); lazy_eq.d_table = d_out; lazy_eq.on = true;
  }
  std::vector<lasso_fr*> gather_tail(const std::vector<lasso_fr*>& polys) {
    const size_t k = polys.size();
    std::vector<lasso_fr> mine(k), all(k * P), col(P);
    d.chk(lasso_read_heads(d.ctx, (const lasso_fr* const*)polys.data(), (uint32_t)k, mine.data()), "lasso_read_heads");
    d.comm.allgather(mine.data(), all.data(), k * sizeof(lasso_fr));
    std::vector<lasso_fr*> out;
    for (size_t i = 0; i < k; i++) {
      for (size_t g = 0; g < P; g++) col[g] = all[g * k + i];
      tail_bufs.emplace_back(d, P);
      d.chk(lasso_upload(d.ctx, tail_bufs.back().p, col.data(), P * sizeof(lasso_fr)), "lasso_upload");
      out.push_back(tail_bufs.back().p);
    }
    return out;
  }

  void arbitrary_rounds(size_t rounds, size_t len, std::vector<lasso_fr*>& polys, size_t combined_degree, bool reduce, SumcheckProof& proof, ScVec& r_out, const std::vector<const uint32_t*>* first_u32 = nullptr) {
    std::vector<const lasso_fr*> cp(polys.begin(), polys.begin() + alpha);
    for (size_t round = 0; round < rounds; round++) {
      std::vector<lasso_fr> ev(combined_degree + 1);
      if (S.spark()) d.chk(lasso_sumcheck_combine_round(d.ctx, &S.abi, cp.data(), polys[alpha], len, (uint32_t)combined_degree, ev.data()), "lasso_sumcheck_combine_round");
      else if (round == 0 && first_u32) d.chk(lasso_sumcheck_combine_round_lt_u32(d.ctx, &S.abi, first_u32->data(), polys[alpha], len, (uint32_t)combined_degree, ev.data()), "lasso_sumcheck_combine_round_lt_u32");
      else d.chk(lasso_sumcheck_combine_round_lt_scaled(d.ctx, &S.abi, cp.data(), polys[alpha], len, (uint32_t)combined_degree, ev.data()), "lasso_sumcheck_combine_round_lt_scaled");
      if (reduce) d.comm.sum(ev);
      ScVec evals; for (auto& e : ev) evals.push_back(Sc::from_abi(e));
      UniPoly up = UniPoly::from_evals(evals);
      up.append_to_transcript(t, "poly");
      Sc r_j = t.challenge_scalar("challenge_nextround"); r_out.push_back(r_j);
      lasso_fr rj = r_j.abi();
      d.chk(lasso_bind_top(d.ctx, polys.data(), (uint32_t)polys.size(), len, &rj), "lasso_bind_top");
      len /= 2;
      proof.compressed_polys.push_back(up.compress());
    }
  }
  void linear_rounds(size_t rounds, size_t len, std::vector<lasso_fr*>& polys, const lasso_fr* d_E, const ScVec& point, size_t v0, bool reduce, Sc& s_run, SumcheckProof& proof, ScVec& r_out,
                     const std::vector<const lasso_fr*>* src = nullptr, std::vector<lasso_fr>* tail_heads = nullptr, const std::vector<const uint32_t*>* src_u32 = nullptr) {
    if (tail_heads) tail_heads->clear();
    if (!rounds) return;
    if (src && rounds < 2) {
      for (size_t i = 0; i < polys.size(); i++) d.chk(lasso_copy(d.ctx, polys[i], (*src)[i], len * sizeof(lasso_fr)), "lasso_copy");
      src = nullptr;
    }
    const ScVec w = S.weights();
    ScVec inv(rounds); bool degenerate = false;
    {
// ... 202 lines not shown
    std::vector<H4> A, B, Aw;
    if (!vec) {
      A.resize(k * m); B.resize(k * m); Aw.resize(k * m);
      for (size_t c = 0; c < k; c++) { const H4 w = h4_from(coeffs[c].v); for (size_t i = 0; i < m; i++) { A[c * m + i] = h4_from(a[c][i].v); B[c * m + i] = h4_from(b[c][i].v); Aw[c * m + i] = h4_mul(A[c * m + i], w); } }
    }
    size_t stride = m;
    for (size_t j = 0; j < rounds_left; j++) {
      const size_t h = m / 2;
      H4 e0 = h4_zero(), e2 = h4_zero(), e3 = h4_zero();
#ifdef LASSO_HOST_IFMA
      if (vec) v52->sums(h, e0, e2, e3); else
#endif
      for (size_t i = 0; i < h; i++) {
        H4 t0 = h4_zero(), t2 = h4_zero(), t3 = h4_zero();
        for (size_t c = 0; c < k; c++) {
          const H4 *pa = &Aw[c * stride], *pb = &B[c * stride];
          const H4 da = h4_sub(pa[i + h], pa[i]), db = h4_sub(pb[i + h], pb[i]), a2 = h4_add(pa[i + h], da), b2 = h4_add(pb[i + h], db), a3 = h4_add(a2, da), b3 = h4_add(b2, db);
          t0 = h4_add(t0, h4_mul(pa[i], pb[i])); t2 = h4_add(t2, h4_mul(a2, b2)); t3 = h4_add(t3, h4_mul(a3, b3));
        }
        const H4 dc = h4_sub(C[i + h], C[i]), c2 = h4_add(C[i + h], dc), c3 = h4_add(c2, dc);
        e0 = h4_add(e0, h4_mul(t0, C[i])); e2 = h4_add(e2, h4_mul(t2, c2)); e3 = h4_add(e3, h4_mul(t3, c3));
      }
      static const H4 inv2 = h4_from(Sc::from_u64(2).inverse().v), inv6 = h4_from(Sc::from_u64(6).inverse().v);
      const H4 e1 = h4_sub(h4_from(e.v), e0);
      const H4 t32 = h4_sub(e3, h4_add(h4_add(e2, e2), e2)), t11 = h4_add(h4_add(e1, e1), e1);
      const H4 k3 = h4_mul(h4_sub(h4_add(t32, t11), e0), inv6);
      const H4 k2 = h4_sub(h4_mul(h4_add(h4_sub(e2, h4_add(e1, e1)), e0), inv2), h4_add(h4_add(k3, k3), k3));
      const H4 k1 = h4_sub(h4_sub(h4_sub(e1, e0), k2), k3);
      UniPoly poly; poly.coeffs = {to_sc(e0), to_sc(k1), to_sc(k2), to_sc(k3)};
      poly.append_to_transcript(t, "poly");
      const Sc r_j = t.challenge_scalar("challenge_nextround"); r_out.push_back(r_j);
      e = poly.evaluate(r_j);
      proof.compressed_polys.push_back(poly.compress());
      const H4 rj = h4_from(r_j.v);
#ifdef LASSO_HOST_IFMA
      if (vec) v52->bind(h, rj); else
#endif
      {
        for (size_t c = 0; c < k; c++) for (H4* arr : {&A[c * stride], &B[c * stride], &Aw[c * stride]}) for (size_t i = 0; i < h; i++) arr[i] = h4_add(arr[i], h4_mul(rj, h4_sub(arr[i + h], arr[i])));
        for (size_t i = 0; i < h; i++) C[i] = h4_add(C[i], h4_mul(rj, h4_sub(C[i + h], C[i])));
      }
      m = h;
    }
    heads.resize(2 * k);
#ifdef LASSO_HOST_IFMA
    if (vec) { std::vector<H4> hh; v52->heads(hh); for (size_t c = 0; c < 2 * k; c++) heads[c] = to_sc(hh[c]).abi(); return; }
#endif
    for (size_t c = 0; c < k; c++) { heads[c] = to_sc(A[c * stride]).abi(); heads[k + c] = to_sc(B[c * stride]).abi(); }
  }
  void cubic_rounds(size_t rounds, size_t len, std::vector<lasso_fr*>& A, std::vector<lasso_fr*>& B, const lasso_fr* d_E, const ScVec& rand, size_t v0, const ScVec& coeffs, bool reduce, Sc& s_run,
                    Sc& e, SumcheckProof& proof, ScVec& r_out, std::vector<lasso_fr>* heads_out = nullptr, const LeafLayer* leaf = nullptr) {
    const size_t k = leaf ? 2 * leaf->mems.size() : A.size();
    if (heads_out) heads_out->clear();
    std::unique_ptr<HostClock> hpro(new HostClock("layer transition: sumcheck prologue"));
    LayerAhead pre = std::move(layer_ahead); layer_ahead.on = false;
    std::function<void()> hook = std::move(next_layer_hook); next_layer_hook = nullptr;
    if (!rounds) { if (pre.on) d.chk(lasso_point_cancel(d.ctx), "lasso_point_cancel"); return; }
    ScVec inv(rounds); bool degenerate = false;
    {
      Sc prod = Sc::one();
      for (size_t j = 0; j < rounds; j++) { Sc om = Sc::one() - rand[v0 + j]; if (om.is_zero()) degenerate = true; prod *= om; }
      if (!degenerate) { Sc pi = prod.inverse(); for (size_t j = rounds; j-- > 0;) { inv[j] = pi; pi *= Sc::one() - rand[v0 + j]; } }
    }
    DBuf tj; if (degenerate) tj = DBuf(d, len / 2);
    Sc r_prev = Sc::zero();
    LazyEq lz; if (lazy_eq.on && lazy_eq.d_table == d_E && v0 == 0) { lz = lazy_eq; } lazy_eq.on = false;
    auto ensure_table = [&] { if (lz.on) { d.chk(lasso_eq_evals_scaled(d.ctx, lz.rr.data(), (uint32_t)lz.rr.size(), &lz.scale, lz.d_table), "lasso_eq_evals_scaled"); lz.on = false; } };
    if (degenerate) lz.on = false;
    static const bool tail_off = [] { const char* v = getenv("LASSO_CUBIC_TAIL"); return v && v[0] == '0'; }();
    size_t tail_from = rounds;
    if (heads_out && !reduce && !degenerate && !tail_off) {
      size_t j0 = 0; size_t l = len;
      while (j0 < rounds && (j0 == 0 ? l / 2 : l / 4) > tail_q()) { if (j0) l /= 2; j0++; }
      bool plain = j0 < rounds;
      for (size_t j = j0; j < rounds && plain; j++) if (rand[v0 + j].is_zero()) plain = false;
      if (plain) tail_from = j0;
    }
    bool in_tail = false;
    size_t m_stop = 1, j_host = rounds;
    if (tail_from < rounds && len == ((size_t)1 << rounds)) {
      const size_t m0 = host_m_stop(k), lt = len >> tail_from;
      if (m0 >= 2 && m0 < lt) { m_stop = m0; j_host = rounds - ceil_log2(m0); }
    }
    bool use_pre = false;
    if (pre.on) {
      static const bool three = [] { const char* v = getenv("LASSO_CUBIC_THREE_SUMS"); return v && v[0] == '1'; }();
      use_pre = lz.on && !degenerate && !leaf && v0 == 0 && heads_out && !reduce && pre.len == len && pre.A == A && pre.B == B && pre.d_table == lz.d_table && pre.ell == lz.rr.size() &&
                (pre.tail ? (tail_from == 0 && m_stop == pre.m_stop) : (tail_from > 0 && !three && !rand[0].is_zero() && !s_run.is_zero()));
      if (!use_pre) d.chk(lasso_point_cancel(d.ctx), "lasso_point_cancel");
    }
    static const bool ahead_env_off = [] { const char* v = getenv("LASSO_ROUNDS_AHEAD"); return v && v[0] == '0'; }();
    static const bool slab_ahead_off = [] { const char* v = getenv("LASSO_SLAB_AHEAD"); return v && v[0] == '0'; }();
    const bool ahead_ok = !ahead_env_off && !degenerate && (reduce ? (!slab_ahead_off && !d.ranks_share_a_device()) : (P == 1 && heads_out != nullptr)) && !d.no_ahead() && lasso_rounds_ahead_ok(d.ctx) == 1;
    bool queued = false, queued_tail = false;
    std::vector<DBuf> leaf_full;
    if (leaf) {
      static const bool three = [] { const char* v = getenv("LASSO_CUBIC_THREE_SUMS"); return v && v[0] == '1'; }();
      const bool plain = v0 == 0 && !degenerate && !three && rounds >= 3 && tail_from >= 2 && !rand[0].is_zero() && !rand[1].is_zero() && !s_run.is_zero();
      if (!plain) { leaf_full = leaf_materialise(*leaf, A, B); leaf = nullptr; }
    }
    hpro.reset();
    for (size_t j = 0; j < j_host; j++) {
      const lasso_fr* table = d_E; Sc scale = degenerate ? Sc::one() : inv[j];
      if (degenerate) {
        std::vector<lasso_fr> rr; for (size_t t2 = v0 + j + 1; t2 < v0 + rounds; t2++) rr.push_back(rand[t2].abi());
        lasso_fr sc = (reduce ? d.comm.eq_low(rand) : Sc::one()).abi();
        d.chk(lasso_eq_evals_scaled(d.ctx, rr.data(), (uint32_t)rr.size(), &sc, tj.p), "lasso_eq_evals_scaled");
        table = tj.p;
      }
      const Sc& rj = rand[v0 + j]; const Sc base = s_run * scale, om = Sc::one() - rj;
      const Sc f0 = base * om, f1 = base * rj;
      UniPoly poly;
      static const bool three_sums = [] { const char* v = getenv("LASSO_CUBIC_THREE_SUMS"); return v && v[0] == '1'; }();
      if (j >= tail_from || queued || (!f1.is_zero() && !three_sums)) {
        lasso_fr rp = r_prev.abi();
        const uint32_t ell = (uint32_t)lz.rr.size();
        std::vector<lasso_fr> ev(2 * k); bool have_ev = false;
        if (queued) {
          d.chk(lasso_challenge_post(d.ctx, &rp), "lasso_challenge_post"); queued = false;
        } else if (queued_tail) {
          d.chk(lasso_sumcheck_cubic_tail_next(d.ctx, &rp), "lasso_sumcheck_cubic_tail_next"); queued_tail = false; in_tail = true;
        } else
        if (j == 0 && use_pre) {
          { HostClock hp("layer transition: point post"); d.chk(lasso_point_post(d.ctx, lz.rr.data(), ell, &lz.scale), "lasso_point_post"); } lz.on = false;
          if (pre.tail) { in_tail = true; if (hook) { hook(); hook = nullptr; } }
        } else
        if (leaf && j < 2) {
          ensure_table();
          leaf_round(*leaf, j, len, table, j ? &rp : nullptr, ev); have_ev = true;
          if (j == 1) { A = leaf->work_a; B = leaf->work_b; }
        } else
        if (j == 0 && lz.on && j < tail_from && ell <= 32 && len / 2 > 64) {
          d.chk(lasso_sumcheck_cubic_eqw2_begin_eq(d.ctx, A.data(), B.data(), (uint32_t)k, lz.d_table, len, lz.rr.data(), ell, &lz.scale), "lasso_sumcheck_cubic_eqw2_begin_eq"); lz.on = false;
        } else if (j == 0 && lz.on && j >= tail_from && ell <= 9) {
          if (m_stop > 1) d.chk(lasso_tail_handover_next(d.ctx, (uint32_t)m_stop), "lasso_tail_handover_next");
          d.chk(lasso_sumcheck_cubic_tail_begin_eq(d.ctx, A.data(), B.data(), (uint32_t)k, len, lz.rr.data(), ell, &lz.scale), "lasso_sumcheck_cubic_tail_begin_eq"); in_tail = true; lz.on = false;
          if (hook) { hook(); hook = nullptr; }
        } else {
          ensure_table();
          if (j < tail_from) d.chk(lasso_sumcheck_cubic_eqw2_begin(d.ctx, A.data(), B.data(), (uint32_t)k, table, len, j == 0 ? nullptr : &rp), "lasso_sumcheck_cubic_eqw2_begin");
          else if (!in_tail) {
            if (m_stop > 1) d.chk(lasso_tail_handover_next(d.ctx, (uint32_t)m_stop), "lasso_tail_handover_next");
            d.chk(lasso_sumcheck_cubic_tail_begin(d.ctx, A.data(), B.data(), (uint32_t)k, table, len, j == 0 ? nullptr : &rp), "lasso_sumcheck_cubic_tail_begin"); in_tail = true;
            if (hook) { hook(); hook = nullptr; }
          }
          else d.chk(lasso_sumcheck_cubic_tail_next(d.ctx, &rp), "lasso_sumcheck_cubic_tail_next");
        }
        if (j) len /= 2;
        if (ahead_ok && !in_tail && !lz.on && j + 1 < j_host && !(leaf && j + 1 < 3) && !rand[v0 + j + 1].is_zero()) {
          if (j + 1 < tail_from) {
            const int32_t rc = lasso_sumcheck_cubic_eqw2_begin_ahead(d.ctx, A.data(), B.data(), (uint32_t)k, table, len);
            if (rc == 0) queued = true; else if (rc != LASSO_ERR_UNSUPPORTED) d.chk(rc, "lasso_sumcheck_cubic_eqw2_begin_ahead");
          } else if (j + 1 == tail_from) {
            if (m_stop > 1) d.chk(lasso_tail_handover_next(d.ctx, (uint32_t)m_stop), "lasso_tail_handover_next");
            d.chk(lasso_sumcheck_cubic_tail_begin_ahead(d.ctx, A.data(), B.data(), (uint32_t)k, table, len), "lasso_sumcheck_cubic_tail_begin_ahead"); queued_tail = true;
            if (hook) { hook(); hook = nullptr; }
          }
        }
        const Sc f1_inv = f1.is_zero() ? Sc::zero() : f1.inverse();
        if (!have_ev) d.chk(lasso_result_wait(d.ctx, ev.data(), 2 * k), "lasso_result_wait");
        if (reduce) d.comm.sum(ev);
        HostClock hc("cubic round host work");
        Sc q0 = Sc::zero(), qi = Sc::zero();
        for (size_t i = 0; i < k; i++) { q0 += Sc::from_abi(ev[2 * i]) * coeffs[i]; qi += Sc::from_abi(ev[2 * i + 1]) * coeffs[i]; }
        const Sc c0 = f0 * q0, q1 = (e - c0) * f1_inv, ql = q1 - q0 - qi, df = f1 - f0;
        poly.coeffs = {c0, f0 * ql + df * q0, f0 * qi + df * ql, df * qi};
      } else {
        std::vector<lasso_fr> ev(3 * k);
        ensure_table();
        if (j == 0) {
          d.chk(lasso_sumcheck_cubic_eqw_round(d.ctx, (const lasso_fr* const*)A.data(), (const lasso_fr* const*)B.data(), (uint32_t)k, table, len, ev.data()), "lasso_sumcheck_cubic_eqw_round");
        } else {
          lasso_fr rp = r_prev.abi();
          d.chk(lasso_sumcheck_cubic_eqw_round_fused(d.ctx, A.data(), B.data(), (uint32_t)k, table, len, &rp, ev.data()), "lasso_sumcheck_cubic_eqw_round_fused");
          len /= 2;
        }
        if (reduce) d.comm.sum(ev);
        const Sc f2 = base * (rj + rj - om), f3 = base * (rj + rj + rj - om - om);
        Sc c0 = Sc::zero(), c2 = Sc::zero(), c3 = Sc::zero();
        for (size_t i = 0; i < k; i++) { c0 += Sc::from_abi(ev[3 * i]) * coeffs[i]; c2 += Sc::from_abi(ev[3 * i + 1]) * coeffs[i]; c3 += Sc::from_abi(ev[3 * i + 2]) * coeffs[i]; }
        c0 *= f0; c2 *= f2; c3 *= f3;
        poly = UniPoly::from_evals({c0, e - c0, c2, c3});
      }
      HostClock hc2("cubic round host work");
      poly.append_to_transcript(t, "poly");
      Sc r_j = t.challenge_scalar("challenge_nextround"); r_out.push_back(r_j);
      r_prev = r_j;
      e = poly.evaluate(r_j);
      s_run *= om * (Sc::one() - r_j) + rj * r_j;
      proof.compressed_polys.push_back(poly.compress());
    }
    lasso_fr rp = r_prev.abi();
    if (in_tail) {
      d.chk(lasso_sumcheck_cubic_tail_next(d.ctx, &rp), "lasso_sumcheck_cubic_tail_next");
      heads_out->resize(2 * k * m_stop);
      d.chk(lasso_result_wait(d.ctx, heads_out->data(), 2 * k * m_stop), "lasso_result_wait");
      if (m_stop > 1) {
        std::vector<ScVec> ha(k, ScVec(m_stop)), hb(k, ScVec(m_stop));
        for (size_t c = 0; c < k; c++) for (size_t i = 0; i < m_stop; i++) { ha[c][i] = Sc::from_abi((*heads_out)[c * m_stop + i]); hb[c][i] = Sc::from_abi((*heads_out)[(k + c) * m_stop + i]); }
        host_cubic_rounds(ha, hb, rounds - j_host, rand, v0 + j_host, coeffs, s_run, e, proof, r_out, *heads_out);
      }
      return;
    }
    LASSO_REQUIRE(j_host == rounds && !queued && !queued_tail);
    std::vector<lasso_fr*> ab(A); ab.insert(ab.end(), B.begin(), B.end());
    d.chk(lasso_bind_top(d.ctx, ab.data(), (uint32_t)ab.size(), len, &rp), "lasso_bind_top");
  }
  SumcheckProof prove_cubic_batched(const Sc& claim, size_t num_rounds, bool slab, std::vector<lasso_fr*>& A, std::vector<lasso_fr*>& B, const lasso_fr* d_E, const ScVec& rand, const ScVec& coeffs,
                                    ScVec& r_out, ScVec& claims_a, ScVec& claims_b, const LeafLayer* leaf = nullptr) {
    SumcheckProof proof; Sc e = claim, s_run = Sc::one(); const size_t k = leaf ? 2 * leaf->mems.size() : A.size();
    LASSO_REQUIRE(rand.size() == num_rounds);
    std::vector<lasso_fr*> fa(A), fb(B);
    std::vector<lasso_fr> heads;
    if (!slab) {
      cubic_rounds(num_rounds, (size_t)1 << num_rounds, fa, fb, d_E, rand, 0, coeffs, false, s_run, e, proof, r_out, &heads, leaf);
    } else {
      LASSO_REQUIRE(num_rounds >= lgP);
      const size_t local_rounds = num_rounds - lgP;
      cubic_rounds(local_rounds, (size_t)1 << local_rounds, fa, fb, d_E, rand, 0, coeffs, true, s_run, e, proof, r_out, nullptr, leaf);
      std::vector<lasso_fr*> local_heads(fa); local_heads.insert(local_heads.end(), fb.begin(), fb.end());
      static const bool slab_host_tail_off = [] { const char* v = getenv("LASSO_SLAB_HOST_TAIL"); return v && v[0] == '0'; }();
      if (!slab_host_tail_off) {
        std::vector<lasso_fr> mine(2 * k), all(2 * k * P);
        d.chk(lasso_read_heads(d.ctx, (const lasso_fr* const*)local_heads.data(), (uint32_t)(2 * k), mine.data()), "lasso_read_heads");
        d.comm.allgather(mine.data(), all.data(), 2 * k * sizeof(lasso_fr));
        std::vector<ScVec> ha(k, ScVec(P)), hb(k, ScVec(P));
        for (size_t g = 0; g < P; g++) for (size_t c = 0; c < k; c++) { ha[c][g] = Sc::from_abi(all[g * 2 * k + c]); hb[c][g] = Sc::from_abi(all[g * 2 * k + k + c]); }
        host_cubic_rounds(ha, hb, lgP, rand, local_rounds, coeffs, s_run, e, proof, r_out, heads);
        claims_a.clear(); claims_b.clear();
        for (size_t i = 0; i < k; i++) { claims_a.push_back(Sc::from_abi(heads[i])); claims_b.push_back(Sc::from_abi(heads[k + i])); }
        return proof;
      }
      std::vector<lasso_fr*> tail = gather_tail(local_heads);
      fa.assign(tail.begin(), tail.begin() + k); fb.assign(tail.begin() + k, tail.begin() + 2 * k);
      tail_bufs.emplace_back(d, P);
      std::vector<lasso_fr> rr; for (size_t i = local_rounds; i < num_rounds; i++) rr.push_back(rand[i].abi());
      d.chk(lasso_eq_evals(d.ctx, rr.data(), (uint32_t)rr.size(), tail_bufs.back().p), "lasso_eq_evals");
      cubic_rounds(lgP, P, fa, fb, tail_bufs.back().p, rand, local_rounds, coeffs, false, s_run, e, proof, r_out, &heads);
    }
    if (heads.empty()) {
      std::vector<lasso_fr*> ab(fa); ab.insert(ab.end(), fb.begin(), fb.end());
      heads.resize(2 * k);
      d.chk(lasso_read_heads(d.ctx, (const lasso_fr* const*)ab.data(), (uint32_t)(2 * k), heads.data()), "lasso_read_heads");
    }
    claims_a.clear(); claims_b.clear();
    for (size_t i = 0; i < k; i++) { claims_a.push_back(Sc::from_abi(heads[i])); claims_b.push_back(Sc::from_abi(heads[k + i])); }
    tail_bufs.clear();
    return proof;
  }
  struct HostTops { size_t len = 0; std::vector<ScVec> run; };
  void enqueue_next_layer(const std::vector<lasso_fr*>& trees, size_t n, size_t layer_id, lasso_fr* d_table) {
    const size_t len = n >> layer_id, off = 2 * n - 2 * len;
    std::vector<lasso_fr*> A, B; for (auto* tr : trees) { A.push_back(tr + off); B.push_back(tr + off + len / 2); }
    enqueue_layer_ahead(A, B, len / 2, d_table);
  }
  BatchedGrandProductArgument bgpa_prove(std::vector<lasso_fr*>& trees, std::vector<lasso_fr*>& tops, size_t n, const ScVec& roots, ScVec& rand_out, LeafLayer* leaf = nullptr, const HostTops* host_tops = nullptr) {
    Trace tr("BatchedGrandProductArgument.prove", d.ctx);
    BatchedGrandProductArgument out; const size_t k = trees.size(), num_layers = ceil_log2(n), n_loc = n / P;
    ScVec claims_to_verify = roots, rand;
    DBuf eq(d, std::max(n_loc / 4, P));
    for (size_t layer_id = num_layers; layer_id-- > 0;) {
      const size_t len = n >> layer_id;
      LASSO_REQUIRE(((size_t)1 << rand.size()) == len / 2);
      const size_t num_rounds_prod = ceil_log2(len / 2);
      if (host_tops && len <= host_tops->len && !(leaf && layer_id == 0)) {
        LASSO_REQUIRE(host_tops->run.size() == k && (P == 1 || host_tops->len == P));
        const size_t off = 2 * host_tops->len - 2 * len;
        std::vector<ScVec> ha(k), hb(k);
        for (size_t c = 0; c < k; c++) { const ScVec& r = host_tops->run[c]; ha[c].assign(r.begin() + off, r.begin() + off + len / 2); hb[c].assign(r.begin() + off + len / 2, r.begin() + off + len); }
        if (P == 1 && layer_id > 0 && 2 * len > host_tops->len && !leaf) enqueue_next_layer(trees, n, layer_id - 1, eq.p);
        ScVec coeff_vec = t.challenge_vector("rand_coeffs_next_layer", claims_to_verify.size());
        Sc claim = Sc::zero(); for (size_t i = 0; i < claims_to_verify.size(); i++) claim += claims_to_verify[i] * coeff_vec[i];
        LayerProofBatched lp; ScVec rand_prod; std::vector<lasso_fr> heads;
        host_cubic_rounds(ha, hb, num_rounds_prod, rand, 0, coeff_vec, Sc::one(), claim, lp.proof, rand_prod, heads);
        for (size_t i = 0; i < k; i++) { lp.claims_prod_left.push_back(Sc::from_abi(heads[i])); lp.claims_prod_right.push_back(Sc::from_abi(heads[k + i])); }
        for (size_t i = 0; i < k; i++) { t.append_scalar("claim_prod_left", lp.claims_prod_left[i]); t.append_scalar("claim_prod_right", lp.claims_prod_right[i]); }
        Sc r_layer = t.challenge_scalar("challenge_r_layer");
        claims_to_verify.clear();
        for (size_t i = 0; i < k; i++) claims_to_verify.push_back(lp.claims_prod_left[i] + r_layer * (lp.claims_prod_right[i] - lp.claims_prod_left[i]));
        ScVec ext{r_layer}; ext.insert(ext.end(), rand_prod.begin(), rand_prod.end()); rand = ext;
        out.proof.push_back(std::move(lp));
        continue;
      }
      const bool slab = P > 1 && len >= 2 * P;
      std::unique_ptr<HostClock> hco(new HostClock("layer transition: opening (arrays, coefficients, claim)"));
      std::vector<lasso_fr*> A, B;
      const bool bottom_leafless = leaf && layer_id == 0;
      if (bottom_leafless) {
        leaf->work_a.clear(); leaf->work_b.clear();
        for (auto* tr : trees) { leaf->work_a.push_back(tr); leaf->work_b.push_back(tr + n_loc / 4); }
        if (eq_inline_off()) eq_half_local(rand, eq.p); else eq_half_lazy(rand, eq.p);
      } else if (slab || P == 1) {
        const size_t len_l = len / P, off = 2 * n_loc - 2 * len_l - (leaf ? n_loc : 0);
        for (auto* tr : trees) { A.push_back(tr + off); B.push_back(tr + off + len_l / 2); }
        if (eq_inline_off()) eq_half_local(rand, eq.p); else eq_half_lazy(rand, eq.p);
      } else {
        const size_t off = 2 * P - 2 * len;
        for (auto* tp : tops) { A.push_back(tp + off); B.push_back(tp + off + len / 2); }
        std::vector<lasso_fr> rr; for (auto& x : rand) rr.push_back(x.abi());
        d.chk(lasso_eq_evals(d.ctx, rr.data(), (uint32_t)rr.size(), eq.p), "lasso_eq_evals");
      }
      ScVec coeff_vec = t.challenge_vector("rand_coeffs_next_layer", claims_to_verify.size());
      Sc claim = Sc::zero(); for (size_t i = 0; i < claims_to_verify.size(); i++) claim += claims_to_verify[i] * coeff_vec[i];
      LayerProofBatched lp; ScVec rand_prod;
      hco.reset();
      next_layer_hook = nullptr;
      if (P == 1 && !leaf && layer_id > 0) next_layer_hook = [this, &trees, n, layer_id, &eq] { enqueue_next_layer(trees, n, layer_id - 1, eq.p); };
      lp.proof = prove_cubic_batched(claim, num_rounds_prod, slab, A, B, eq.p, rand, coeff_vec, rand_prod, lp.claims_prod_left, lp.claims_prod_right, bottom_leafless ? leaf : nullptr);
      next_layer_hook = nullptr;
      HostClock hcl("layer transition: closing claims + r_layer");
      for (size_t i = 0; i < k; i++) { t.append_scalar("claim_prod_left", lp.claims_prod_left[i]); t.append_scalar("claim_prod_right", lp.claims_prod_right[i]); }
      Sc r_layer = t.challenge_scalar("challenge_r_layer");
      claims_to_verify.clear();
      for (size_t i = 0; i < k; i++) claims_to_verify.push_back(lp.claims_prod_left[i] + r_layer * (lp.claims_prod_right[i] - lp.claims_prod_left[i]));
      ScVec ext{r_layer}; ext.insert(ext.end(), rand_prod.begin(), rand_prod.end()); rand = ext;
      out.proof.push_back(std::move(lp));
    }
    rand_out = rand; return out;
  }

  Pt msm_dev(const PolyCommitmentGens& g, const lasso_fr* d_scalars, size_t n) {
    lasso_point out; d.chk(lasso_msm_dev(d.ctx, g.bases, d_scalars, n, &out), "lasso_msm_dev");
    return Pt::from_abi(out);
  }
  DotProductProofLog dot_product_log_prove(const PolyCommitmentGens& g, DBuf& d_a0, DBuf& d_b0, const std::vector<uint8_t>& a_bytes, const Sc& y) {
    static_assert(sizeof(Sc) == sizeof(lasso_fr), "ScVec is uploaded as an array of lasso_fr");
    Trace tr("DotProductProofLog.prove", d.ctx);
    t.append_protocol_name("dot product proof (log)");
    const size_t n = g.n; LASSO_REQUIRE(d_a0.n == n && d_b0.n == n && a_bytes.size() == 32 * n);
    const size_t lg_n = ceil_log2(n);
    Sc dd, r_delta, r_beta; ScVec v1, v2;
    {
      HostClock hc("opening: random tape");
      dd = tape.random_scalar("d"); r_delta = tape.random_scalar("r_delta"); r_beta = tape.random_scalar("r_delta");
      v1 = tape.random_vector("blinds_vec_1", 2 * lg_n); v2 = tape.random_vector("blinds_vec_2", 2 * lg_n);
    }
    const bool shard = d.comm.sharded() && g.slab_open;
    const uint32_t cw = (uint32_t)d.comm.world, cr = (uint32_t)d.comm.rank;
    auto sum_points = [&](const lasso_point* mine, size_t count, Pt* out) {
      std::vector<lasso_point> all(count * cw);
      d.comm.allgather(mine, all.data(), count * sizeof(lasso_point));
      for (size_t i = 0; i < count; i++) { Pt acc = Pt::from_abi(all[i]); for (size_t r2 = 1; r2 < cw; r2++) acc = acc + Pt::from_abi(all[r2 * count + i]); out[i] = acc; }
    };
    DotProductProofLog P; uint8_t buf[32];
    DBuf d_a1(d, n / 2 ? n / 2 : 1), d_b1(d, n / 2 ? n / 2 : 1), d_w0(d, n), d_w1(d, n);
    d.chk(lasso_eq_evals(d.ctx, nullptr, 0, d_w0.p), "lasso_eq_evals");
    {
      lasso_point cx;
      d.chk(lasso_defer_next(d.ctx), "lasso_defer_next");
      if (shard) d.chk(lasso_msm_dev_slab(d.ctx, g.bases_slab, d_a0.p, n, cw, cr, nullptr, nullptr, &cx), "lasso_msm_dev_slab");
      else d.chk(lasso_msm_dev(d.ctx, g.bases, d_a0.p, n, &cx), "lasso_msm_dev");
      uint8_t cy[32]; compress_one(g.Qmul.mul(y), cy);
      d.chk(lasso_result_wait(d.ctx, (lasso_fr*)&cx, 4), "lasso_result_wait");
      Pt cxp = Pt::from_abi(cx); if (shard) sum_points(&cx, 1, &cxp);
      compress_one(cxp, buf); t.append_point_bytes("Cx", buf);
      t.append_point_bytes("Cy", cy);
    }
    lasso_fr *a_cur = d_a0.p, *a_nxt = d_a1.p, *b_cur = d_b0.p, *b_nxt = d_b1.p, *w_cur = d_w0.p, *w_nxt = d_w1.p;
    Sc blind_fin = Sc::zero(); size_t nk = n, nw = 1, round = 0;
    bool have_u = false; lasso_fr ua, uia;
    const bool ahead = !shard && !d.no_ahead() && lasso_bullet_ahead_ok(d.ctx, g.bases) == 1;
    bool queued = false;
    const bool tail_ahead = ahead && lasso_bullet_tail_ahead_ok(d.ctx, g.bases) == 1;
    bool tail_queued = false;
    auto enqueue_tail = [&](size_t nw_now) {
      lasso_fr sc = dd.abi(); lasso_fr tl[2] = {Sc::zero().abi(), r_delta.abi()};
      const int32_t rc = lasso_bullet_tail_ahead(d.ctx, g.bases, n, a_cur, b_cur, w_cur, nw_now, w_nxt, &sc, tl);
      if (rc == 0) { std::swap(w_cur, w_nxt); tail_queued = true; } else if (rc != LASSO_ERR_UNSUPPORTED) d.chk(rc, "lasso_bullet_tail_ahead");
    };
    auto enqueue_next = [&](size_t nk_next) {
      lasso_fr bl[2] = {v1[round + 1].abi(), v2[round + 1].abi()};
      d.chk(lasso_bullet_round_ahead(d.ctx, g.bases, n, a_cur, b_cur, w_cur, a_nxt, b_nxt, w_nxt, nk_next, bl), "lasso_bullet_round_ahead");
      std::swap(a_cur, a_nxt); std::swap(b_cur, b_nxt); std::swap(w_cur, w_nxt);
      queued = true;
    };
    while (nk != 1) {
      const Sc& blind_L = v1[round]; const Sc& blind_R = v2[round];
      lasso_fr blinds[2] = {blind_L.abi(), blind_R.abi()};
      lasso_point LR[2];
      if (have_u && queued) {
        d.chk(lasso_bullet_post(d.ctx, &ua, &uia), "lasso_bullet_post");
        queued = false;
        if (nk / 2 != 1) enqueue_next(nk / 2); else if (tail_ahead) enqueue_tail(nw);
        d.chk(lasso_result_wait(d.ctx, (lasso_fr*)LR, 8), "lasso_result_wait");
      } else if (have_u) {
        if (shard) d.chk(lasso_bullet_round_slab(d.ctx, g.bases_slab, n, cw, cr, a_cur, b_cur, w_cur, a_nxt, b_nxt, w_nxt, nk, &ua, &uia, blinds, LR), "lasso_bullet_round_slab");
        else d.chk(lasso_bullet_round(d.ctx, g.bases, n, a_cur, b_cur, w_cur, a_nxt, b_nxt, w_nxt, nk, &ua, &uia, blinds, LR), "lasso_bullet_round");
        std::swap(a_cur, a_nxt); std::swap(b_cur, b_nxt); std::swap(w_cur, w_nxt);
      } else {
        d.chk(lasso_defer_next(d.ctx), "lasso_defer_next");
// ... 440 lines not shown
```

Before: 1.113 billion.

## Split next-layer eq point into high/low classes to start first-round sumcheck early

Adds a layer-classes path for the grand-product sumcheck. Once the high part of the next layer's random point is known (after the device tail rounds), the high eq table is posted and the first cubic round is computed as 2^b class sums per circuit. When the low challenges arrive, the host folds those class sums with a small eq over the low bits, and the full eq table is built behind a second gate. The goal is to overlap the next layer's first-round evaluation with the host's remaining rounds and cut layer-transition latency, at the cost of extra gate/mailbox logic, extra partials and host combination work.

Measured after the change: 1.115 billion, median of 3. About the same (+0.2%).

```diff
diff --git a/lasso_amd/csrc/lasso_hip.hip b/lasso_amd/csrc/lasso_hip.hip
--- a/lasso_amd/csrc/lasso_hip.hip
+++ b/lasso_amd/csrc/lasso_hip.hip
@@ -11,6 +11,7 @@
 #include <cstdlib>
 #include <ctime>
 #include "../../include/lasso_hip.h"
+#include "lasso_layer_classes.h"
 #include "poly_kernels.cuh"
 #include "msm_kernels.cuh"
 #include "densify_kernels.cuh"
@@ -60,6 +61,7 @@
   uint32_t* pmail_h = nullptr; uint32_t* pmail_d = nullptr; uint32_t* d_gpoint = nullptr;
   uint32_t gate_sent = 0;
   bool lay_active = false, lay_tail = false, lay_tagged = false, no_grow = false; uint32_t lay_seq = 0, lay_ell = 0, lay_groups = 1, lay_K = 0, lay_turns = 0; size_t lay_count = 0, lay_final = 0;
+  bool lay_cls = false; uint32_t cls_stage = 0, cls_seq_h = 0, cls_seq_l = 0, cls_seq_r = 0, cls_b = 0, cls_ell_h = 0;
   uint32_t prof_mask = 0;
   std::vector<EventPair> events; size_t events_used = 0;
   uint64_t prof_launches[LASSO_K_COUNT] = {0}; double prof_ms[LASSO_K_COUNT] = {0}; double prof_bytes[LASSO_K_COUNT] = {0};
@@ -450,7 +452,7 @@
   (void)hipGetLastError();
   if (c->pmail_h) { memset(c->pmail_h, 0, LASSO_PMAIL_BYTES); c->gate_sent = 0; }
   mail_chunks(c->mail_h + 12, 0, zero8); post_mail(c, 0, zero8);
-  c->lay_active = false; c->lay_tail = false; c->no_grow = false;
+  c->lay_active = false; c->lay_tail = false; c->lay_cls = false; c->cls_stage = 0; c->no_grow = false;
   c->ahead_active = false; c->ahead_bullet = false; c->tail_unstarted = false; c->handover_next = 0;
   c->tail_active = false; c->pending = false; c->defer_next = false; c->events_used = 0; c->pending_groups = 1; c->pending_K = 0;
   HIPCHK(c, hipMemsetAsync(c->d_counters, 0, (LASSO_MAX_PTRS + 40) * 4, c->stream));
@@ -832,12 +834,12 @@
   if (rc == LASSO_ERR_UNSUPPORTED) return fail(c, rc, "lasso_sumcheck_cubic_tail_begin_eq_ahead: a buffer would have to grow while kernels are in flight");
   return rc;
 }
-static void point_mail(lasso_ctx* c, uint32_t ell, const lasso_fr* point, const lasso_fr* scale, uint32_t ctrl) {
+static void point_mail(lasso_ctx* c, uint32_t ell, const lasso_fr* point, const lasso_fr* scale, uint32_t ctrl, uint32_t seq) {
   const uint32_t zero8[8] = {0, 0, 0, 0, 0, 0, 0, 0}; const fr_t one = fr_one();
-  for (uint32_t j = 0; j < ell; j++) mail_chunks(c->pmail_h + 12 * j, c->lay_seq, point ? (const uint32_t*)(point + j) : zero8);
-  mail_chunks(c->pmail_h + 12 * ell, c->lay_seq, scale ? (const uint32_t*)scale : one.v);
+  for (uint32_t j = 0; j < ell; j++) mail_chunks(c->pmail_h + 12 * j, seq, point ? (const uint32_t*)(point + j) : zero8);
+  mail_chunks(c->pmail_h + 12 * ell, seq, scale ? (const uint32_t*)scale : one.v);
   const uint32_t ctl[8] = {ctrl, 0, 0, 0, 0, 0, 0, 0};
-  mail_chunks(c->pmail_h + 12 * (ell + 1), c->lay_seq, ctl);
+  mail_chunks(c->pmail_h + 12 * (ell + 1), seq, ctl);
 #if defined(__SSE2__)
   _mm_sfence();
 #else
@@ -845,8 +847,8 @@
 #endif
 }
 int32_t lasso_point_post(lasso_ctx* c, const lasso_fr* point, uint32_t ell, const lasso_fr* scale) {
-  REQUIRE(c, c && c->lay_active && ell == c->lay_ell && (point || !ell) && !c->pending && !c->tail_active && !c->ahead_active);
-  point_mail(c, ell, point, scale, 0u);
+  REQUIRE(c, c && c->lay_active && !c->lay_cls && ell == c->lay_ell && (point || !ell) && !c->pending && !c->tail_active && !c->ahead_active);
+  point_mail(c, ell, point, scale, 0u, c->lay_seq);
   c->lay_active = false;
   if (c->lay_tail) {
     c->tail_active = true; c->tail_seq0 = c->lay_seq; c->tail_turn = 0; c->tail_turns = c->lay_turns; c->tail_count = c->lay_count; c->tail_final = c->lay_final; c->tail_unstarted = false;
@@ -859,8 +861,98 @@
 }
 int32_t lasso_point_cancel(lasso_ctx* c) {
   REQUIRE(c, c && c->lay_active);
-  point_mail(c, c->lay_ell, nullptr, nullptr, 1u);
+  if (c->lay_cls) return lasso_layer_classes_cancel(c);
+  point_mail(c, c->lay_ell, nullptr, nullptr, 1u, c->lay_seq);
   c->lay_active = false; c->lay_tail = false;
+  return 0;
+}
+static unsigned cls_nx(size_t half, uint32_t ncirc) { return grid_for(half, cubic_nx_cap(ncirc)); }
+int32_t lasso_layer_classes_ahead(lasso_ctx* c, lasso_fr* const* d_A, lasso_fr* const* d_B, uint32_t ncirc, lasso_fr* d_E_out, size_t n, uint32_t ell, uint32_t b) {
+  REQUIRE(c, c && d_A && d_B && d_E_out && ncirc >= 1 && ncirc <= LASSO_MAX_PTRS && n >= 2 && (n & (n - 1)) == 0 && ell < 48 && ((size_t)1 << ell) == n / 2 && b <= 6 && b < ell &&
+             !c->lay_active && !c->ahead_active && !c->defer_next);
+  if (!lasso_layer_ahead_ok(c) || !c->tagged || n / 2 <= CUBIC_SMALL_Q || ell > 32 || ell - b + 2 > LASSO_POINT_MAX + 2) return fail(c, LASSO_ERR_UNSUPPORTED, "lasso_layer_classes_ahead: streaming layers with tagged results only");
+  if (!gate_free(c)) return fail(c, LASSO_ERR_UNSUPPORTED, "lasso_layer_classes_ahead: the previous point gate has not consumed its message yet");
+  for (uint32_t i = 0; i < ncirc; i++) REQUIRE(c, d_A[i] && d_B[i]);
+  const size_t half = n / 2; const uint32_t C = 1u << b, K = 2 * C, ell_h = ell - b, h_lo = ell_h / 2, h_hi = ell_h - h_lo;
+  const unsigned ny = ncirc, nx = cls_nx(half, ncirc);
+  const size_t part_elems = (size_t)nx * ny * K, fac = ((size_t)1 << h_hi) + ((size_t)1 << h_lo), h_elems = b ? 0 : ((size_t)1 << ell_h);
+  c->no_grow = true;
+  int32_t rc = ensure_small(c, (size_t)ncirc * K);
+  if (!rc) rc = ensure_scratch(c, (part_elems + fac + h_elems) * sizeof(fr_t));
+  c->no_grow = false;
+  if (rc == LASSO_ERR_UNSUPPORTED) return fail(c, rc, "lasso_layer_classes_ahead: a buffer would have to grow while kernels are in flight");
+  if (rc) return rc;
+  fr_t* const partials = (fr_t*)c->d_scratch; fr_t* const f_hi = partials + part_elems; fr_t* const f_lo = f_hi + ((size_t)1 << h_hi);
+  fr_t* const H = b ? (fr_t*)d_E_out + n / 4 : f_lo + ((size_t)1 << h_lo);
+  const uint32_t seq_h = next_seq(c, 3), seq_r = seq_h + 1, seq_l = seq_h + 2;
+  uint32_t* const ack = c->pmail_d + LASSO_PMAIL_ACK_WORD; const uint32_t* const gp = c->d_gpoint;
+  hipLaunchKernelGGL(k_gate_point, dim3(1), dim3(64), 0, c->stream, (const uint32_t*)c->pmail_d, c->d_gpoint, seq_h, ell_h + 2u, ack);
+  {
+    ProfScope pe(c, LASSO_K_EQ, 32.0 * (double)(((size_t)1 << ell_h) + fac));
+    const unsigned hb = grid_for((size_t)1 << h_hi), lb = grid_for((size_t)1 << h_lo);
+    hipLaunchKernelGGL(k_eq_small2_mem, dim3(hb + lb), dim3(LASSO_BLOCK), 0, c->stream, gp, seq_h, h_hi, f_hi, hb, h_lo, f_lo);
+    hipLaunchKernelGGL(k_eq_outer, dim3(grid_for((size_t)1 << ell_h, 4096)), dim3(LASSO_BLOCK), 0, c->stream, (const fr_t*)f_hi, (const fr_t*)f_lo, h_lo, (size_t)1 << ell_h, H, gp, seq_h);
+  }
+  {
+    ProfScope ps(c, LASSO_K_CUBIC, 32.0 * n * (2.0 * ncirc + 1.0));
+    if (ncirc <= 8) {
+      PtrTable8 Ac, Bc; for (uint32_t i = 0; i < ncirc; i++) { Ac.p[i] = (const fr_t*)d_A[i]; Bc.p[i] = (const fr_t*)d_B[i]; }
+      hipLaunchKernelGGL((k_cubic_eqw_cls<PtrTable8>), dim3(nx * ny), dim3(LASSO_BLOCK), 0, c->stream, Ac, Bc, nx, ny, (const fr_t*)H, b, half, partials, gp, seq_h);
+    } else {
+      PtrTable Ac, Bc; for (uint32_t i = 0; i < ncirc; i++) { Ac.p[i] = (const fr_t*)d_A[i]; Bc.p[i] = (const fr_t*)d_B[i]; }
+      hipLaunchKernelGGL((k_cubic_eqw_cls<PtrTable>), dim3(nx * ny), dim3(LASSO_BLOCK), 0, c->stream, Ac, Bc, nx, ny, (const fr_t*)H, b, half, partials, gp, seq_h);
+    }
+    hipLaunchKernelGGL(k_cls_reduce, dim3(ny * K), dim3(LASSO_BLOCK), 0, c->stream, (const fr_t*)partials, nx, (fr_t*)c->d_tag, seq_r, gp, seq_h);
+  }
+  hipLaunchKernelGGL(k_gate_point_after, dim3(1), dim3(64), 0, c->stream, (const uint32_t*)c->pmail_d, c->d_gpoint, seq_l, b + 2u, ack, seq_h);
+  {
+    ProfScope pe(c, LASSO_K_EQ, 32.0 * (double)(n / 4));
+    hipLaunchKernelGGL(k_eq_cls_table, dim3(grid_for(n / 4, 4096)), dim3(LASSO_BLOCK), 0, c->stream, (const fr_t*)H, b, n / 4, (fr_t*)d_E_out, gp, seq_l);
+  }
+  HIPCHK(c, hipGetLastError());
+  c->gate_sent = seq_l;
+  c->lay_active = true; c->lay_tail = false; c->lay_cls = true; c->cls_stage = 0; c->cls_seq_h = seq_h; c->cls_seq_r = seq_r; c->cls_seq_l = seq_l; c->cls_b = b; c->cls_ell_h = ell_h;
+  c->lay_seq = seq_h; c->lay_ell = ell; c->lay_count = (size_t)ncirc * K; c->lay_tagged = true;
+  return 0;
+}
+int32_t lasso_layer_classes_post_hi(lasso_ctx* c, const lasso_fr* point_hi) {
+  REQUIRE(c, c && c->lay_active && c->lay_cls && c->cls_stage == 0 && (point_hi || !c->cls_ell_h));
+  point_mail(c, c->cls_ell_h, point_hi, nullptr, 0u, c->cls_seq_h);
+  c->cls_stage = 1;
+  return 0;
+}
+static int32_t cls_wait_first_gate(lasso_ctx* c, bool& ok) {
+  const double t0 = now_us(); uint64_t spins = 0;
+  for (;;) {
+    const uint32_t a = __atomic_load_n(c->pmail_h + LASSO_PMAIL_ACK_WORD, __ATOMIC_ACQUIRE);
+    if (a == c->cls_seq_h) { ok = true; return 0; }
+    if (a == c->cls_seq_l) { ok = false; return 0; }
+    if ((++spins & 0xffff) == 0) {
+      const hipError_t q = hipStreamQuery(c->stream);
+      if (q != hipSuccess && q != hipErrorNotReady) return fail(c, LASSO_ERR_HIP, std::string("stream error while waiting for a point gate: ") + hipGetErrorString(q));
+      if (now_us() - t0 > 20e6) return fail(c, LASSO_ERR_HIP, "a point gate did not acknowledge its message");
+    }
+    __builtin_ia32_pause();
+  }
+}
+int32_t lasso_layer_classes_post_lo(lasso_ctx* c, const lasso_fr* point_lo, const lasso_fr* scale) {
+  REQUIRE(c, c && c->lay_active && c->lay_cls && c->cls_stage == 1 && (point_lo || !c->cls_b) && !c->pending && !c->tail_active && !c->ahead_active);
+  bool ok = false; int32_t rc = cls_wait_first_gate(c, ok); if (rc) return rc;
+  c->lay_active = false; c->lay_cls = false;
+  if (!ok) return fail(c, LASSO_ERR_HIP, "lasso_layer_classes_post_lo: the layer's first point gate failed (5 s without its message)");
+  point_mail(c, c->cls_b, point_lo, scale, 0u, c->cls_seq_l);
+  c->pending = true; c->pending_seq = c->cls_seq_r; c->pending_count = c->lay_count; c->pending_tagged = true; c->pending_groups = 1; c->pending_K = 0;
+  c->cls_stage = 0;
+  return 0;
+}
+int32_t lasso_layer_classes_wait(lasso_ctx* c, lasso_fr* out, size_t count) { return lasso_result_wait(c, out, count); }
+int32_t lasso_layer_classes_cancel(lasso_ctx* c) {
+  REQUIRE(c, c && c->lay_active && c->lay_cls);
+  c->lay_active = false; c->lay_cls = false;
+  if (c->cls_stage == 0) { point_mail(c, c->cls_ell_h, nullptr, nullptr, 1u, c->cls_seq_h); return 0; }
+  bool ok = false; int32_t rc = cls_wait_first_gate(c, ok); if (rc) return rc;
+  if (ok) point_mail(c, c->cls_b, nullptr, nullptr, 1u, c->cls_seq_l);
+  c->cls_stage = 0;
   return 0;
 }
 int32_t lasso_sumcheck_cubic_tail_begin_ahead(lasso_ctx* c, lasso_fr* const* d_A, lasso_fr* const* d_B, uint32_t ncirc, const lasso_fr* d_E, size_t n) {
diff --git a/lasso_amd/csrc/lasso_layer_classes.h b/lasso_amd/csrc/lasso_layer_classes.h
--- /dev/null
+++ b/lasso_amd/csrc/lasso_layer_classes.h
@@ -0,0 +1,15 @@
+#pragma once
+#include <stddef.h>
+#include <stdint.h>
+#include "../../include/lasso_hip.h"
+#ifdef __cplusplus
+extern "C" {
+#endif
+int32_t lasso_layer_classes_ahead(lasso_ctx* c, lasso_fr* const* d_A, lasso_fr* const* d_B, uint32_t ncirc, lasso_fr* d_E_out, size_t n, uint32_t ell, uint32_t b);
+int32_t lasso_layer_classes_post_hi(lasso_ctx* c, const lasso_fr* point_hi);
+int32_t lasso_layer_classes_post_lo(lasso_ctx* c, const lasso_fr* point_lo, const lasso_fr* scale);
+int32_t lasso_layer_classes_wait(lasso_ctx* c, lasso_fr* out, size_t count);
+int32_t lasso_layer_classes_cancel(lasso_ctx* c);
+#ifdef __cplusplus
+}
+#endif
diff --git a/lasso_amd/csrc/poly_kernels.cuh b/lasso_amd/csrc/poly_kernels.cuh
--- a/lasso_amd/csrc/poly_kernels.cuh
+++ b/lasso_amd/csrc/poly_kernels.cuh
@@ -151,7 +151,7 @@
 #define LASSO_PMAIL_BYTES 2048
 #define LASSO_GPOINT_BYTES 2048
 #define LASSO_PMAIL_ACK_WORD 504
-__global__ void __launch_bounds__(64) k_gate_point(const uint32_t* pmail, uint32_t* gpoint, uint32_t seq, uint32_t nfr, uint32_t* ack) {
+__device__ __forceinline__ void gate_point_body(const uint32_t* pmail, uint32_t* gpoint, uint32_t seq, uint32_t nfr, uint32_t* ack) {
   const uint32_t t = threadIdx.x;
   const uint64_t t_end = wall_clock64() + 500000000ull;
   bool ok = true; fr_t v = fr_zero();
@@ -166,6 +166,14 @@
   const bool all_ok = __ballot(!ok) == 0;
   __builtin_amdgcn_fence(__ATOMIC_RELEASE, "agent");
   if (t == 0) { gpoint[LASSO_GP_TAG + (all_ok ? 0 : 1)] = seq; if (ack) __hip_atomic_store(ack, seq, __ATOMIC_RELEASE, __HIP_MEMORY_SCOPE_SYSTEM); }
+}
+__global__ void __launch_bounds__(64) k_gate_point(const uint32_t* pmail, uint32_t* gpoint, uint32_t seq, uint32_t nfr, uint32_t* ack) { gate_point_body(pmail, gpoint, seq, nfr, ack); }
+__global__ void __launch_bounds__(64) k_gate_point_after(const uint32_t* pmail, uint32_t* gpoint, uint32_t seq, uint32_t nfr, uint32_t* ack, uint32_t prev) {
+  if (!(gpoint[LASSO_GP_TAG] == prev && gpoint[LASSO_GP_TAG + 1] != prev)) {
+    if (threadIdx.x == 0) { gpoint[LASSO_GP_TAG + 1] = seq; __hip_atomic_store(ack, seq, __ATOMIC_RELEASE, __HIP_MEMORY_SCOPE_SYSTEM); }
+    return;
+  }
+  gate_point_body(pmail, gpoint, seq, nfr, ack);
 }
 __device__ __forceinline__ bool gate_point_ok(const uint32_t* __restrict__ gp, uint32_t seq) { return gp[LASSO_GP_TAG] == seq && gp[LASSO_GP_TAG + 1] != seq; }
 __device__ __forceinline__ fr_t gate_point_fr(const uint32_t* __restrict__ gp, uint32_t j) {
@@ -428,6 +436,87 @@
   if (NT == 2) { fr29_acc_carry(w0); fr29_acc_carry(w1); e[0] = fr29_acc_reduce(w0); e[1] = fr29_acc_reduce(w1); }
   cubic_epilogue(e, g, partials, counters, out, flag, seq, S, 5, NT);
 }
+template <class TP>
+__global__ void __launch_bounds__(LASSO_BLOCK) k_cubic_eqw_cls(TP A, TP B, uint32_t nx, uint32_t ny, const fr_t* __restrict__ H, uint32_t cb, size_t half, fr_t* __restrict__ partials,
+                                                                const uint32_t* __restrict__ gp, uint32_t gseq) {
+  __shared__ RedScratch S;
+  if (!gate_point_ok(gp, gseq)) return;
+  const CubicGrid g = cubic_grid(nx, ny);
+  const fr_t* __restrict__ a = A.p[g.by];
+  const fr_t* __restrict__ b = B.p[g.by];
+  fr29_acc w0 = fr29_acc_zero(), w1 = fr29_acc_zero(); uint32_t cnt = 0;
+  const size_t stride = (size_t)nx * blockDim.x;
+  size_t i = g.bx * (size_t)blockDim.x + threadIdx.x;
+  if (i < half) {
+    fr_t a0 = a[i], a1 = a[i + half], b0m = b[i], b1m = b[i + half], em = H[i >> cb];
+    for (;;) {
+      const size_t in = i + stride; const bool more = in < half;
+      const size_t ip = more ? in : i;
+      const fr_t na0 = a[ip], na1 = a[ip + half], nb0 = b[ip], nb1 = b[ip + half], ne = H[ip >> cb];
+      const fr29 es = fr29_unpack_s(em), b0 = fr29_unpack_u(b0m), b1 = fr29_unpack_u(b1m);
+      const fr29 g0 = fr29_mul(fr29_unpack_u(a0), es), g1 = fr29_mul(fr29_unpack_u(a1), es);
+      fr29_mul_acc(w0, b0, g0); fr29_mul_acc(w1, fr29_sub(g1, g0), fr29_sub(b1, b0));
+      if (++cnt == 3) { fr29_acc_carry(w0); fr29_acc_carry(w1); cnt = 0; }
+      if (!more) break;
+      a0 = na0; a1 = na1; b0m = nb0; b1m = nb1; em = ne; i = in;
+    }
+  }
+  fr29_acc_carry(w0); fr29_acc_carry(w1);
+  const fr29 e0 = fr29_acc_reduce(w0), e1 = fr29_acc_reduce(w1);
+  const uint32_t t = threadIdx.x, C = 1u << cb, K = 2 * C, R = LASSO_BLOCK >> cb, ncol = 9 * K;
+#pragma unroll
+  for (int k = 0; k < 9; k++) { S.rows[t * 27 + k] = e0.v[k]; S.rows[t * 27 + 9 + k] = e1.v[k]; }
+  __syncthreads();
+  uint32_t P = 1; while (2 * P * ncol <= LASSO_BLOCK && 2 * P <= R) P *= 2;
+  const uint32_t W = ncol * P, rp = R / P;
+  int64_t part[5];
+#pragma unroll
+  for (int it = 0; it < 5; it++) {
+    const uint32_t w = t + LASSO_BLOCK * it; int64_t s = 0;
+    if (w < W) {
+      const uint32_t col = w / P, p = w - col * P, u = col / 9, k = col - u * 9, v = u >> cb, x = u & (C - 1);
+      for (uint32_t m = p * rp; m < (p + 1) * rp; m++) s += S.rows[(x + (m << cb)) * 27 + v * 9 + k];
+    }
+    part[it] = s;
+  }
+  __syncthreads();
+  int64_t* T = reinterpret_cast<int64_t*>(S.rows);
+#pragma unroll
+  for (int it = 0; it < 5; it++) { const uint32_t w = t + LASSO_BLOCK * it; if (w < W) T[w] = part[it]; }
+  __syncthreads();
+  if (t < K) {
+    int64_t c[9];
+#pragma unroll
+    for (int k = 0; k < 9; k++) { int64_t s = 0; for (uint32_t p = 0; p < P; p++) s += T[(t * 9 + k) * P + p]; c[k] = s; }
+    partials[((size_t)g.by * K + t) * nx + g.bx] = fr29_pack(fr29_reduce_columns(c, 5));
+  }
+}
+__global__ void __launch_bounds__(LASSO_BLOCK) k_cls_reduce(const fr_t* __restrict__ partials, uint32_t nx, fr_t* __restrict__ out, uint32_t seq, const uint32_t* __restrict__ gp, uint32_t gseq) {
+  __shared__ RedScratch S;
+  if (!gate_point_ok(gp, gseq)) return;
+  const size_t row = blockIdx.x;
+  fr29 acc[1] = {fr29_zero()}; uint32_t cnt = 0;
+  for (uint32_t x = threadIdx.x; x < nx; x += blockDim.x) acc_add(acc[0], fr29_unpack_u(partials[row * nx + x]), cnt);
+  block_columns<1>(acc, S);
+  if (threadIdx.x == 0) {
+    result_store(out, row, columns_to_fr(S, 0, 0), LASSO_TAGGED, seq);
+    __builtin_amdgcn_fence(__ATOMIC_RELEASE, "");
+  }
+}
+__global__ void __launch_bounds__(LASSO_BLOCK) k_eq_cls_table(const fr_t* __restrict__ H, uint32_t cb, size_t n, fr_t* __restrict__ out, const uint32_t* __restrict__ gp, uint32_t gseq) {
+  __shared__ fr29 sl[64];
+  if (!gate_point_ok(gp, gseq)) return;
+  const uint32_t t = threadIdx.x;
+  if (t < (1u << cb)) {
+    fr29 p = fr29_unpack_u(gate_point_fr(gp, cb));
+    const fr29 one_s = fr29_one_s();
+    for (uint32_t j = 0; j < cb; j++) { const bool bit = (t >> (cb - 1 - j)) & 1u; const fr29 rs = fr29_unpack_s(gate_point_fr(gp, j)); p = fr29_mul(bit ? rs : fr29_sub(one_s, rs), p); }
+    sl[t] = fr29_unpack_s(fr29_store(p));
+  }
+  __syncthreads();
+  const size_t mask = ((size_t)1 << cb) - 1;
+  for (size_t x = blockIdx.x * (size_t)blockDim.x + t; x < n; x += (size_t)gridDim.x * blockDim.x) out[x] = fr29_store(fr29_mul(fr29_unpack_u(H[x >> cb]), sl[x & mask]));
+}
 template <int NT, bool WIDE = false, class TM = MutPtrTable, bool AHEAD = false>
 #ifdef LASSO_FUSED_WAVES
 __attribute__((amdgpu_waves_per_eu(LASSO_FUSED_WAVES, LASSO_FUSED_WAVES)))
diff --git a/lasso_amd/host/prover.hpp b/lasso_amd/host/prover.hpp
--- a/lasso_amd/host/prover.hpp
+++ b/lasso_amd/host/prover.hpp
@@ -8,6 +8,8 @@
 #include "field_host.hpp"
 #include "field52.hpp"
 #include "hashes.hpp"
+#include "../csrc/lasso_layer_classes.h"
+#include <dlfcn.h>
 #include "../../include/lasso_prover.h"
 
 #include <chrono>
@@ -627,11 +629,30 @@
   std::vector<DBuf> side_keep;
   static size_t tail_q() { static const size_t q = lasso_sumcheck_tail_capacity(); return q; }
   struct LazyEq { bool on = false; std::vector<lasso_fr> rr; lasso_fr scale; lasso_fr* d_table = nullptr; } lazy_eq;
-  struct LayerAhead { bool on = false, tail = false; std::vector<lasso_fr*> A, B; lasso_fr* d_table = nullptr; size_t len = 0, m_stop = 1; uint32_t ell = 0; } layer_ahead;
+  struct LayerAhead { bool on = false, tail = false, cls = false, hi_posted = false; std::vector<lasso_fr*> A, B; lasso_fr* d_table = nullptr; size_t len = 0, m_stop = 1; uint32_t ell = 0, b = 0; std::vector<lasso_fr> hi; } layer_ahead;
   std::function<void()> next_layer_hook;
+  int hook_cls_b = -1;
+  struct ClassFns {
+    decltype(&lasso_layer_classes_ahead) ahead = nullptr; decltype(&lasso_layer_classes_post_hi) post_hi = nullptr; decltype(&lasso_layer_classes_post_lo) post_lo = nullptr;
+    decltype(&lasso_layer_classes_wait) wait = nullptr; decltype(&lasso_layer_classes_cancel) cancel = nullptr;
+    bool ok() const { return ahead && post_hi && post_lo && wait && cancel; }
+  };
+  static const ClassFns& class_fns() {
+    static const ClassFns f = [] {
+      ClassFns r; Dl_info info;
+      if (!dladdr((void*)&lasso_ctx_create, &info) || !info.dli_fname) return r;
+      void* h = dlopen(info.dli_fname, RTLD_NOW | RTLD_NOLOAD); if (!h) return r;
+      r.ahead = (decltype(r.ahead))dlsym(h, "lasso_layer_classes_ahead"); r.post_hi = (decltype(r.post_hi))dlsym(h, "lasso_layer_classes_post_hi");
+      r.post_lo = (decltype(r.post_lo))dlsym(h, "lasso_layer_classes_post_lo"); r.wait = (decltype(r.wait))dlsym(h, "lasso_layer_classes_wait");
+      r.cancel = (decltype(r.cancel))dlsym(h, "lasso_layer_classes_cancel");
+      dlclose(h); return r;
+    }();
+    return f;
+  }
+  static bool layer_classes_on() { static const bool v = [] { const char* e = getenv("LASSO_LAYER_CLASSES"); return !(e && e[0] == '0') && class_fns().ok(); }(); return v; }
   static bool tail_switched_off() { static const bool off = [] { const char* v = getenv("LASSO_CUBIC_TAIL"); return v && v[0] == '0'; }(); return off; }
   bool layer_ahead_ok() { return P == 1 && !d.no_ahead() && !eq_inline_off() && !tail_switched_off() && lasso_layer_ahead_ok(d.ctx) == 1; }
-  void enqueue_layer_ahead(const std::vector<lasso_fr*>& A, const std::vector<lasso_fr*>& B, size_t len, lasso_fr* d_table) {
+  void enqueue_layer_ahead(const std::vector<lasso_fr*>& A, const std::vector<lasso_fr*>& B, size_t len, lasso_fr* d_table, int cls_b = -1) {
     layer_ahead.on = false;
     if (!layer_ahead_ok() || len < 4) return;
     const size_t k = A.size(); const uint32_t ell = (uint32_t)ceil_log2(len / 2);
@@ -644,7 +665,12 @@
       rc = lasso_sumcheck_cubic_tail_begin_eq_ahead(d.ctx, la.A.data(), la.B.data(), (uint32_t)k, len, ell);
     } else {
       if (ell > 32 || len / 2 <= 64) return;
-      rc = lasso_sumcheck_cubic_eqw2_begin_eq_ahead(d.ctx, la.A.data(), la.B.data(), (uint32_t)k, d_table, len, ell);
+      rc = LASSO_ERR_UNSUPPORTED;
+      if (cls_b >= 0 && cls_b <= 6 && (uint32_t)cls_b < ell && layer_classes_on()) {
+        rc = class_fns().ahead(d.ctx, la.A.data(), la.B.data(), (uint32_t)k, d_table, len, ell, (uint32_t)cls_b);
+        if (rc == 0) { la.cls = true; la.b = (uint32_t)cls_b; } else if (rc != LASSO_ERR_UNSUPPORTED) d.chk(rc, "lasso_layer_classes_ahead");
+      }
+      if (!la.cls) rc = lasso_sumcheck_cubic_eqw2_begin_eq_ahead(d.ctx, la.A.data(), la.B.data(), (uint32_t)k, d_table, len, ell);
     }
     if (rc == LASSO_ERR_UNSUPPORTED) return;
     d.chk(rc, "lasso_sumcheck_cubic_*_begin_eq_ahead");
@@ -1013,11 +1039,13 @@
       const size_t m0 = host_m_stop(k), lt = len >> tail_from;
       if (m0 >= 2 && m0 < lt) { m_stop = m0; j_host = rounds - ceil_log2(m0); }
     }
+    hook_cls_b = (tail_from < rounds && v0 == 0 && !reduce) ? (int)(rounds - j_host) : -1;
     bool use_pre = false;
     if (pre.on) {
       static const bool three = [] { const char* v = getenv("LASSO_CUBIC_THREE_SUMS"); return v && v[0] == '1'; }();
       use_pre = lz.on && !degenerate && !leaf && v0 == 0 && heads_out && !reduce && pre.len == len && pre.A == A && pre.B == B && pre.d_table == lz.d_table && pre.ell == lz.rr.size() &&
-                (pre.tail ? (tail_from == 0 && m_stop == pre.m_stop) : (tail_from > 0 && !three && !rand[0].is_zero() && !s_run.is_zero()));
+                (pre.tail ? (tail_from == 0 && m_stop == pre.m_stop) : (tail_from > 0 && !three && !rand[0].is_zero() && !s_run.is_zero())) &&
+                (!pre.cls || (pre.hi_posted && pre.b < lz.rr.size() && pre.hi.size() == lz.rr.size() - pre.b && !memcmp(pre.hi.data(), lz.rr.data(), pre.hi.size() * sizeof(lasso_fr))));
       if (!use_pre) d.chk(lasso_point_cancel(d.ctx), "lasso_point_cancel");
     }
     static const bool ahead_env_off = [] { const char* v = getenv("LASSO_ROUNDS_AHEAD"); return v && v[0] == '0'; }();
@@ -1046,11 +1074,14 @@
       if (j >= tail_from || queued || (!f1.is_zero() && !three_sums)) {
         lasso_fr rp = r_prev.abi();
         const uint32_t ell = (uint32_t)lz.rr.size();
-        std::vector<lasso_fr> ev(2 * k); bool have_ev = false;
+        std::vector<lasso_fr> ev(2 * k); bool have_ev = false, cls_wait = false;
         if (queued) {
           d.chk(lasso_challenge_post(d.ctx, &rp), "lasso_challenge_post"); queued = false;
         } else if (queued_tail) {
           d.chk(lasso_sumcheck_cubic_tail_next(d.ctx, &rp), "lasso_sumcheck_cubic_tail_next"); queued_tail = false; in_tail = true;
+        } else
+        if (j == 0 && use_pre && pre.cls) {
+          { HostClock hp("layer transition: point post"); d.chk(class_fns().post_lo(d.ctx, lz.rr.data() + (ell - pre.b), &lz.scale), "lasso_layer_classes_post_lo"); } lz.on = false; cls_wait = true;
         } else
         if (j == 0 && use_pre) {
           { HostClock hp("layer transition: point post"); d.chk(lasso_point_post(d.ctx, lz.rr.data(), ell, &lz.scale), "lasso_point_post"); } lz.on = false;
@@ -1089,6 +1120,19 @@
           }
         }
         const Sc f1_inv = f1.is_zero() ? Sc::zero() : f1.inverse();
+        if (cls_wait) {
+          const size_t b = pre.b, C = (size_t)1 << b, eh = ell - b;
+          std::vector<lasso_fr> cs(2 * k * C);
+          d.chk(class_fns().wait(d.ctx, cs.data(), cs.size()), "lasso_layer_classes_wait");
+          HostClock hcc("layer transition: class sums");
+          ScVec lo(b); for (size_t t2 = 0; t2 < b; t2++) lo[t2] = Sc::from_abi(lz.rr[eh + t2]);
+          const std::vector<H4> sl = eq_evals_host_scaled(lo.data(), b, Sc::from_abi(lz.scale));
+          for (size_t i = 0; i < 2 * k; i++) {
+            Sc acc = Sc::zero();
+            for (size_t x = 0; x < C; x++) { Sc w; w.v = h4_to(sl[x]); acc += w * Sc::from_abi(cs[i * C + x]); }
+            ev[i] = acc.abi();
+          }
+        } else
         if (!have_ev) d.chk(lasso_result_wait(d.ctx, ev.data(), 2 * k), "lasso_result_wait");
         if (reduce) d.comm.sum(ev);
         HostClock hc("cubic round host work");
@@ -1124,6 +1168,11 @@
     lasso_fr rp = r_prev.abi();
     if (in_tail) {
       d.chk(lasso_sumcheck_cubic_tail_next(d.ctx, &rp), "lasso_sumcheck_cubic_tail_next");
+      if (layer_ahead.on && layer_ahead.cls && !layer_ahead.hi_posted && v0 == 0 && r_out.size() == j_host && layer_ahead.ell == rounds && layer_ahead.b == rounds - j_host) {
+        std::vector<lasso_fr> hi; for (const Sc& x : r_out) hi.push_back(x.abi());
+        { HostClock hp("layer transition: point post (H)"); d.chk(class_fns().post_hi(d.ctx, hi.data()), "lasso_layer_classes_post_hi"); }
+        layer_ahead.hi = std::move(hi); layer_ahead.hi_posted = true;
+      }
       heads_out->resize(2 * k * m_stop);
       d.chk(lasso_result_wait(d.ctx, heads_out->data(), 2 * k * m_stop), "lasso_result_wait");
       if (m_stop > 1) {
@@ -1180,10 +1229,10 @@
     return proof;
   }
   struct HostTops { size_t len = 0; std::vector<ScVec> run; };
-  void enqueue_next_layer(const std::vector<lasso_fr*>& trees, size_t n, size_t layer_id, lasso_fr* d_table) {
+  void enqueue_next_layer(const std::vector<lasso_fr*>& trees, size_t n, size_t layer_id, lasso_fr* d_table, int cls_b = -1) {
     const size_t len = n >> layer_id, off = 2 * n - 2 * len;
     std::vector<lasso_fr*> A, B; for (auto* tr : trees) { A.push_back(tr + off); B.push_back(tr + off + len / 2); }
-    enqueue_layer_ahead(A, B, len / 2, d_table);
+    enqueue_layer_ahead(A, B, len / 2, d_table, cls_b);
   }
   BatchedGrandProductArgument bgpa_prove(std::vector<lasso_fr*>& trees, std::vector<lasso_fr*>& tops, size_t n, const ScVec& roots, ScVec& rand_out, LeafLayer* leaf = nullptr, const HostTops* host_tops = nullptr) {
     Trace tr("BatchedGrandProductArgument.prove", d.ctx);
@@ -1236,7 +1285,7 @@
       LayerProofBatched lp; ScVec rand_prod;
       hco.reset();
       next_layer_hook = nullptr;
-      if (P == 1 && !leaf && layer_id > 0) next_layer_hook = [this, &trees, n, layer_id, &eq] { enqueue_next_layer(trees, n, layer_id - 1, eq.p); };
+      if (P == 1 && !leaf && layer_id > 0) next_layer_hook = [this, &trees, n, layer_id, &eq] { enqueue_next_layer(trees, n, layer_id - 1, eq.p, hook_cls_b); };
       lp.proof = prove_cubic_batched(claim, num_rounds_prod, slab, A, B, eq.p, rand, coeff_vec, rand_prod, lp.claims_prod_left, lp.claims_prod_right, bottom_leafless ? leaf : nullptr);
       next_layer_hook = nullptr;
       HostClock hcl("layer transition: closing claims + r_layer");
```
